# astomodynamics/cddp-cpp

Measured on AMD Instinct MI355X. Metric: trajectories_per_sec, higher is better.
Workload: dtype f64

## Files before the change

cddp-cpp_amd/csrc/capi.hip:

```cpp
#include <algorithm>
#include <chrono>
#include <cmath>
#include <cstdarg>
#include <cstdio>
#include <cstdlib>
#include <cstring>
#include <string>
#include <vector>
#include <map>

#include "launch.hpp"
#include "plant.hpp"
#include "io_kernels.hpp"

static int ladder_strictly_decreasing(const double *a, int n) {
  for (int i = 1; i < n; ++i) if (!(a[i] < a[i - 1])) return 0;
  return n > 0 ? 1 : 0;
}

using namespace cddp_dev;

namespace cddp_dev {
static __global__ void k_gather_records(DevBuf d, cddp_hip_gather_record *out) {
  const int b = blockIdx.x * blockDim.x + threadIdx.x;
// ... 79 lines not shown
  for (int i = 0; i < nu; ++i) Ulog[((size_t)b * steps + k) * nu + i] = Uc[(((size_t)0 * NB + tile) * nu + i) * 64 + lane];
  for (int i = 0; i < nx; ++i) Xlog[((size_t)b * (steps + 1) + k + 1) * nx + i] = Xc[(((size_t)1 * NB + tile) * nx + i) * 64 + lane];
  itlog[(size_t)b * steps + k] = d.iter[b]; stlog[(size_t)b * steps + k] = d.status[b];
}

static __global__ void k_mark_cpu_time(DevBuf d) {
  const int b = blockIdx.x * blockDim.x + threadIdx.x;
  if (b >= d.B || d.phase[b] == PH_DONE) return;
  d.iter[b] += 1; d.status[b] = CDDP_HIP_STATUS_MAX_CPU_TIME; d.phase[b] = PH_DONE;
}

}

int cddp_host_model_eval(int model, int integrator, double dt, const double *params, int nx, int nu, const double *x, const double *u, double *x_next,
                         double *fx, double *fu, double *fxx, double *fuu, double *fux, std::string &err);
int cddp_host_model_params(int model, int nx, int nu, const double *in, double *out, std::string &err);

namespace {

thread_local std::string g_err;
int fail(int code, const char *fmt, ...) {
  char buf[1024];
  va_list ap; va_start(ap, fmt); vsnprintf(buf, sizeof(buf), fmt, ap); va_end(ap);
  g_err = buf;
  return code;
}
}
extern "C" int cddp_hip_internal_set_error(int code, const char *msg) { g_err = msg ? msg : ""; return code; }
extern "C" int cddp_hip_internal_allgather(const void *send, void *recv, size_t bytes_per_rank, void *comm, void *stream);
namespace {
#define HIPCHK(expr)                                                                          \
  do { hipError_t e_ = (expr); if (e_ != hipSuccess)                                           \
      return fail(-10, "%s failed: %s (%s:%d)", #expr, hipGetErrorString(e_), __FILE__, __LINE__); } while (0)

const std::vector<KernelSet> &registry() {
  static std::vector<KernelSet> v = [] {
    std::vector<KernelSet> r;
    register_pendulum(r); register_cartpole(r); register_unicycle(r); register_lti(r);
    register_quadrotor(r); register_quad12(r); register_manipulator(r); register_manip7(r); register_terminal(r); register_statebox(r);
    register_vehicles(r); register_spacecraft(r); register_plants_small(r); register_plants_nx10(r);
    return r;
  }();
  return v;
}

}

struct CuSpec { int lo[3] = {-1, -1, -1}, hi[3] = {-1, -1, -1}; unsigned xcd[3] = {0, 0, 0}; };
struct CuPlan {
  hipStream_t fwd = nullptr, sweep = nullptr;
  hipEvent_t ev[6] = {nullptr, nullptr, nullptr, nullptr, nullptr, nullptr};
  SweepHop hop{nullptr, nullptr, nullptr};
};

struct Inner {
  ProblemDev P;
  DevBuf d;
  const KernelSet *ks = nullptr;
  const Knobs *knob = nullptr;
  Route route;
  int device = 0;
  hipStream_t stream = nullptr;
  bool own_stream = false;
  CuPlan cu;
  std::vector<void *> allocs;
  ProblemDev *dP = nullptr;
  double *d_xref_traj = nullptr;
  unsigned long long *d_launched = nullptr;
  double *d_Xinit = nullptr, *d_Uinit = nullptr;
  bool have_initial = false;
  bool initialized = false;
  bool has_state = false;
  bool initial_dirty = false;
  bool ms_cache_started = false;
  size_t bytes = 0;
  int timing_detail = CDDP_HIP_TIMING_ROLLOUT;
  std::vector<hipEvent_t> ev_pool;
  hipEvent_t ev_begin = nullptr, ev_end = nullptr, ev_poll = nullptr, ev_poll2 = nullptr;
  double *d_head = nullptr, *h_head = nullptr; size_t head_cap = 0;
  int *h_poll = nullptr;
  std::map<unsigned long long, hipGraphExec_t> graphs;
  bool shadow_bufs = false;
  int cs_epoch = 0;
  int n_redo = 0;
  bool last_shadow = false;
  bool ever_solved = false;
  int *h_bad = nullptr;
  bool has_plan = false;
  double *d_xnext = nullptr;
  double *d_log_u = nullptr, *d_log_x = nullptr; int32_t *d_log_it = nullptr, *d_log_st = nullptr; int log_steps = 0;
};

namespace {

template <class T>
int dalloc(Inner *h, T **p, size_t n) {
  if (n == 0) n = 1;
  void *q = nullptr;
  HIPCHK(hipMalloc(&q, n * sizeof(T)));
  HIPCHK(hipMemsetAsync(q, 0, n * sizeof(T), h->stream));
  h->allocs.push_back(q);
  h->bytes += n * sizeof(T);
  *p = (T *)q;
  return 0;
}

int pool_put(ProblemDev &P, int &top, const double *src, int n) {
  if (top + n > kPool) return -1;
  int off = top;
  for (int i = 0; i < n; ++i) P.pool[off + i] = src[i];
  top += n;
  return off;
}

bool model_has_hessians(int model) {
  return model == CDDP_HIP_MODEL_PENDULUM || model == CDDP_HIP_MODEL_CARTPOLE || model == CDDP_HIP_MODEL_UNICYCLE || model == CDDP_HIP_MODEL_LTI ||
         model == CDDP_HIP_MODEL_BICYCLE || model == CDDP_HIP_MODEL_CAR || model == CDDP_HIP_MODEL_MANIPULATOR || model == CDDP_HIP_MODEL_HCW ||
         model == CDDP_HIP_MODEL_QUADROTOR || model == CDDP_HIP_MODEL_QUADROTOR_EULER12 || model == CDDP_HIP_MODEL_MANIPULATOR7 ||
         model == CDDP_HIP_MODEL_EULER_ATTITUDE || model == CDDP_HIP_MODEL_QUATERNION_ATTITUDE || model == CDDP_HIP_MODEL_MRP_ATTITUDE ||
         model == CDDP_HIP_MODEL_SPACECRAFT_LANDING2D ||
         model == CDDP_HIP_MODEL_DUBINS_CAR || model == CDDP_HIP_MODEL_DREYFUS_ROCKET || model == CDDP_HIP_MODEL_ACROBOT || model == CDDP_HIP_MODEL_USV_3DOF ||
         model == CDDP_HIP_MODEL_FORKLIFT || model == CDDP_HIP_MODEL_SPACECRAFT_LINEAR_FUEL || model == CDDP_HIP_MODEL_QUADROTOR_RATE;
}

int fail_no_hessians(int model) {
  if (model == CDDP_HIP_MODEL_SPACECRAFT_NONLINEAR) return fail(-3, "use_ilqr=false: %s", SpacecraftNonlinearModel::kNoHessMsg);
  if (model == CDDP_HIP_MODEL_SPACECRAFT_TWOBODY) return fail(-3, "use_ilqr=false: %s", SpacecraftTwobodyModel::kNoHessMsg);
  return fail(-3, "use_ilqr=false needs the plant's Hessian tensors, which model id %d does not have", model);
}

int flatten(const cddp_hip_problem *p, ProblemDev &P) {
  std::memset(&P, 0, sizeof(P));
  if (p->abi_version != CDDP_HIP_ABI_VERSION) return fail(-2, "ABI version mismatch: got %d want %d", p->abi_version, CDDP_HIP_ABI_VERSION);
  if (p->nx <= 0 || p->nu <= 0 || p->horizon <= 0 || !(p->dt > 0)) return fail(-2, "bad dimensions nx=%d nu=%d N=%d dt=%g", p->nx, p->nu, p->horizon, p->dt);
  if (!p->Q || !p->R || !p->Qf || !p->x_ref) return fail(-2, "objective matrices (Q, R, Qf, x_ref) must be set before solving");
  if (p->solver != CDDP_HIP_SOLVER_CLDDP && p->solver != CDDP_HIP_SOLVER_IPDDP && p->solver != CDDP_HIP_SOLVER_LOGDDP && p->solver != CDDP_HIP_SOLVER_MSIPDDP)
    return fail(-2, "UnknownSolver - No solver registered for id %d", p->solver);
  if (p->solver == CDDP_HIP_SOLVER_MSIPDDP && p->n_constraints > 0 && !(p->nu == 1 || p->nx == p->nu))
    return fail(-3, "MSIPDDP with path constraints is only defined for nu = 1 or nx = nu: the reference adds an (nx x nu) product to its (nu x nx) block Q_ux (msipddp_solver.cpp:1398)");
  if (p->solver == CDDP_HIP_SOLVER_LOGDDP && !(p->options.logddp_relaxed_delta > 0.0))
    return fail(-2, "Relaxation delta must be positive.");
  if (!(p->options.reg_update_factor > 1.0) || !(p->options.reg_max_value > 0.0))
    return fail(-2, "regularization.update_factor must be > 1 and max_value > 0 (got %g, %g)", p->options.reg_update_factor, p->options.reg_max_value);
  if (!p->options.use_ilqr && !model_has_hessians(p->model)) return fail_no_hessians(p->model);
  P.solver = p->solver; P.model = p->model; P.integrator = p->integrator;
  P.nx = p->nx; P.nu = p->nu; P.N = p->horizon; P.dt = p->dt; P.opt = p->options;
  P.ls_rule = p->options.enable_parallel ? CDDP_HIP_LS_BEST_MERIT : CDDP_HIP_LS_FIRST_SUCCESS;
  {
    std::string err;
    if (cddp_host_model_params(p->model, p->nx, p->nu, p->model_params, P.mp, err)) return fail(-2, "%s", err.c_str());
  }
  if (p->model == CDDP_HIP_MODEL_CAR) P.mp[1] = p->dt;
  if (p->model == CDDP_HIP_MODEL_FORKLIFT) P.mp[3] = p->dt;
  if (p->model == CDDP_HIP_MODEL_LTI) {
    if (!p->lti_A || !p->lti_B) return fail(-2, "LTI model needs lti_A and lti_B");
    if (p->nx * p->nx + p->nx * p->nu + 1 > 32) return fail(-3, "LTI dims too large for the device parameter block");
    for (int i = 0; i < p->nx * p->nx; ++i) P.mp[i] = p->lti_A[i];
    for (int i = 0; i < p->nx * p->nu; ++i) P.mp[p->nx * p->nx + i] = p->lti_B[i];
    P.mp[p->nx * p->nx + p->nx * p->nu] = p->dt;
  }
  int top = 0;
  {
    std::vector<double> q((size_t)p->nx * p->nx), r((size_t)p->nu * p->nu);
    for (size_t i = 0; i < q.size(); ++i) q[i] = p->Q[i] * p->dt;
    for (size_t i = 0; i < r.size(); ++i) r[i] = p->R[i] * p->dt;
    P.off_Qdt = pool_put(P, top, q.data(), (int)q.size());
// ... 288 lines not shown
  }
  h->device = device;
  hipError_t e = hipSetDevice(device);
  if (e != hipSuccess) { delete h; return fail(-10, "hipSetDevice: %s", hipGetErrorString(e)); }
  e = make_stream(&h->stream, device, cu ? cu->lo[0] : -1, cu ? cu->hi[0] : -1, cu ? cu->xcd[0] : 0);
  if (e != hipSuccess) { delete h; return fail(-10, "hipStreamCreate: %s", hipGetErrorString(e)); }
  h->own_stream = true;
  if (cu && (cu->lo[1] >= 0 || cu->lo[2] >= 0)) {
    if (cu->lo[1] >= 0) e = make_stream(&h->cu.fwd, device, cu->lo[1], cu->hi[1], cu->xcd[1]);
    if (e == hipSuccess && cu->lo[2] >= 0) e = make_stream(&h->cu.sweep, device, cu->lo[2], cu->hi[2], cu->xcd[2]);
    for (int k = 0; k < 6 && e == hipSuccess; ++k) e = hipEventCreateWithFlags(&h->cu.ev[k], hipEventDisableTiming);
    if (e != hipSuccess) { const int rc_ = fail(-10, "CU-masked stream: %s", hipGetErrorString(e)); in_destroy(h); return rc_; }
    h->cu.hop = SweepHop{h->cu.sweep, h->cu.ev[4], h->cu.ev[5]};
  }

  const ProblemDev &P = h->P;
  DevBuf &d = h->d;
  std::memset(&d, 0, sizeof(d));
  const int B = batch, Bp = (batch + 63) / 64 * 64, N = P.N, nx = P.nx, nu = P.nu, m = P.m;
  d.B = B; d.Bp = Bp; d.NB = Bp / 64; d.N = N; d.n_alphas = P.n_alphas; d.n_slots = P.n_alphas + 1;
  d.ladder_sorted = ladder_strictly_decreasing(P.alphas, P.n_alphas);
  d.ddp = P.opt.use_ilqr ? 0 : 1;
  d.fail_costate_mask = knob.fail_costate;
  d.xcd_map = knob.xcd_map ? 1 : 0;
  d.hist_batch = P.opt.return_iteration_info ? std::min(B, 64) : 0;
  d.hist_cap = std::max(P.opt.max_iterations, 0) + 1;
  d.planeX = (size_t)(N + 1) * nx * Bp; d.planeU = (size_t)N * nu * Bp; d.planeM = (size_t)N * (m > 0 ? m : 0) * Bp;
  const bool ip = (P.solver == CDDP_HIP_SOLVER_IPDDP);
  d.lg = (P.solver == CDDP_HIP_SOLVER_LOGDDP) ? 1 : 0;
  const bool ms = (P.solver == CDDP_HIP_SOLVER_MSIPDDP);
  d.ms = ms ? 1 : 0;
  d.filt_cap = ms ? std::max(P.opt.max_iterations, 0) + 2 : kFilterCap;
#define DA(ptr, n) do { int rc_ = dalloc(h, &(ptr), (size_t)(n)); if (rc_) { in_destroy(h); return rc_; } } while (0)
  DA(d.X, d.planeX * d.n_slots); DA(d.U, d.planeU * d.n_slots);
  if (ip) { DA(d.S, d.planeM * d.n_slots); DA(d.Y, d.planeM * d.n_slots); DA(d.G, d.planeM * d.n_slots); DA(d.Lam, d.planeX * d.n_slots); }
  if (ms) {
    if (m > 0) { DA(d.S, d.planeM * d.n_slots); DA(d.Y, d.planeM * d.n_slots); DA(d.G, d.planeM * d.n_slots);
                 DA(d.ks, (size_t)N * m * Bp); DA(d.ky, (size_t)N * m * Bp); DA(d.Ks, (size_t)N * m * nx * Bp); DA(d.Ky, (size_t)N * m * nx * Bp); }
    DA(d.Lam, d.planeX * d.n_slots); DA(d.F, d.planeX * d.n_slots);
    DA(d.kl, (size_t)N * nx * Bp);
    if (m == 0) DA(d.fac, (size_t)N * (nu * nu + nu + 1) * Bp);
    if (m > 0) { DA(d.ms_res, (size_t)3 * Bp); DA(d.ev, (size_t)d.n_slots * N * P.n_cons * Bp); }
    if (m > 0 && h->ks->ms_cst_size > 0) DA(d.cst, (size_t)N * h->ks->ms_cst_size * Bp);
  }
  DA(d.A, (size_t)N * nx * nx * Bp); DA(d.Bm, (size_t)N * nx * nu * Bp);
  DA(d.K, (size_t)N * nu * nx * Bp); DA(d.k, (size_t)N * nu * Bp);
  if (ip && nx > 8) DA(d.Kt, (size_t)N * (nu * nx + nu) * Bp);
  DA(d.Vx, (size_t)(N + 1) * nx * Bp); DA(d.Vxx, (size_t)(N + 1) * nx * nx * Bp);
  if (ip && h->ks->cst_size > 0) { DA(d.cst, (size_t)N * h->ks->cst_size * Bp); DA(d.dX, (size_t)N * nx * Bp); DA(d.ys, (size_t)N * (m > 0 ? m : 1) * Bp); }
  if (ip && m > 0) { DA(d.ks, (size_t)N * m * Bp); DA(d.ky, (size_t)N * m * Bp); DA(d.Ks, (size_t)N * m * nx * Bp); DA(d.Ky, (size_t)N * m * nx * Bp); }
  double **scal[] = {&d.cost, &d.merit, &d.inf_pr, &d.inf_du, &d.inf_comp, &d.step_norm, &d.alpha_pr, &d.alpha_du, &d.reg, &d.mu,
                     &d.dV0, &d.dV1, &d.phi, &d.theta, &d.filter_theta, &d.apr_max, &d.adu_max};
  for (double **sp : scal) DA(*sp, Bp);
  DA(d.filt, (size_t)2 * d.filt_cap * Bp);
  int **iscal[] = {&d.filt_n, &d.iter, &d.status, &d.phase, &d.cur, &d.n_bwd, &d.n_fwd, &d.bwd_ok};
  for (int **sp : iscal) DA(*sp, Bp);
  double **tr[] = {&d.t_cost, &d.t_merit, &d.t_theta, &d.t_inf_pr, &d.t_inf_comp, &d.t_apr, &d.t_adu, &d.t_ysmin, &d.t_ysmax};
  for (double **sp : tr) DA(*sp, (size_t)d.n_alphas * Bp);
  DA(d.sink, kSinkDoubles);
  DA(d.t_success, (size_t)d.n_alphas * Bp);
  DA(d.t_steps, (size_t)d.n_alphas * Bp); DA(d.n_fwd_steps, Bp); DA(d.cand, Bp);
  if (ip && P.n_cons > 0) DA(d.ev, (size_t)d.n_alphas * N * 2 * P.n_cons * Bp);
  if (d.lg && P.n_cons > 0) DA(d.ev, (size_t)d.n_slots * N * P.n_cons * Bp);
  DA(d.hist, (size_t)std::max(1, d.hist_batch) * d.hist_cap * kHistCols);
  DA(d.hist_n, std::max(1, d.hist_batch));
  if (ip && P.n_term > 0) {
    DA(d.ST, (size_t)8 * Bp); DA(d.YT, (size_t)8 * Bp); DA(d.GT, (size_t)8 * Bp); DA(d.dST, (size_t)8 * Bp); DA(d.dYT, (size_t)8 * Bp);
    DA(d.LamT, (size_t)16 * Bp); DA(d.dLamT, (size_t)16 * Bp);
    DA(d.STt, (size_t)d.n_alphas * 8 * Bp); DA(d.YTt, (size_t)d.n_alphas * 8 * Bp); DA(d.GTt, (size_t)d.n_alphas * 8 * Bp);
    DA(d.LamTt, (size_t)d.n_alphas * 16 * Bp);
    if (P.pT > 0) {
      const bool te_coop = h->ks->te_rec_size > 0 && P.mT == 0 && P.pT + 1 <= h->ks->te_group && P.pT <= P.nx;
      const size_t nv = te_coop ? 16 : (size_t)(P.pT + 1);
      DA(d.te_k, nv * N * nu * Bp); DA(d.te_p, nv * (N + 1) * nx * Bp);
      if (te_coop) {
        DA(d.te_cst, (size_t)N * h->ks->te_rec_size * Bp); DA(d.te_cnt, Bp);
        if (!d.dX) DA(d.dX, (size_t)N * nx * Bp);
        if (!d.ys) DA(d.ys, (size_t)N * (m > 0 ? m : 1) * Bp);
      }
    }
  }
  DA(d.n_active, 1);
  DA(d.win_hist, CDDP_HIP_MAX_ALPHAS + 1);
  DA(h->d_launched, 1);
  DA(h->dP, 1);
  DA(h->d_Xinit, d.planeX); DA(h->d_Uinit, d.planeU);
  if (problem->x_ref_traj) {
    DA(h->d_xref_traj, (size_t)(N + 1) * nx);
    hipMemcpyAsync(h->d_xref_traj, problem->x_ref_traj, sizeof(double) * (N + 1) * nx, hipMemcpyHostToDevice, h->stream);
    d.xref_traj = h->d_xref_traj;
  }
#undef DA
  hipMemcpyAsync(h->dP, &h->P, sizeof(ProblemDev), hipMemcpyHostToDevice, h->stream);
  d.P = h->dP;
  d.launched = h->d_launched;
  resolve_route(h);
  if (shadow_layout(h) && knob.costate != Knobs::kCostateSync && !knob.fail_costate && !knob.graph) {
#define DA(ptr, n) do { int rc_ = dalloc(h, &(ptr), (size_t)(n)); if (rc_) { in_destroy(h); return rc_; } } while (0)
    DA(d.Vx2, (size_t)(N + 1) * nx * Bp); DA(d.Vxx2, (size_t)(N + 1) * nx * nx * Bp);
    DA(d.cs_stampv, Bp); DA(d.cs_old, Bp); DA(d.cs_new, Bp); DA(d.cs_apr, Bp); DA(d.cs_vbuf, Bp); DA(d.cs_bad, 1);
#undef DA
    if (hipHostMalloc((void **)&h->h_bad, sizeof(int)) != hipSuccess) { const int rc_ = fail(-10, "hipHostMalloc failed"); in_destroy(h); return rc_; }
    *h->h_bad = 0;
    h->shadow_bufs = true;
  }
  e = hipStreamSynchronize(h->stream);
  if (e != hipSuccess) { const int rc_ = fail(-10, "device initialisation failed: %s", hipGetErrorString(e)); in_destroy(h); return rc_; }
  *out = h;
  return 0;
}

static int in_destroy(Inner *h) {
  if (h) { for (auto &kv : h->graphs) hipGraphExecDestroy(kv.second); h->graphs.clear(); }
  if (!h) return 0;
  hipSetDevice(h->device);
  hipStreamSynchronize(h->stream);
  if (h->cu.fwd) hipStreamSynchronize(h->cu.fwd);
  if (h->cu.sweep) hipStreamSynchronize(h->cu.sweep);
  free_all(h);
  for (hipEvent_t e : h->ev_pool) hipEventDestroy(e);
  if (h->ev_begin) { hipEventDestroy(h->ev_begin); hipEventDestroy(h->ev_end); }
  if (h->ev_poll) hipEventDestroy(h->ev_poll);
  if (h->ev_poll2) hipEventDestroy(h->ev_poll2);
  if (h->h_poll) hipHostFree(h->h_poll);
  if (h->h_bad) hipHostFree(h->h_bad);
  if (h->d_head) hipFree(h->d_head);
  if (h->h_head) hipHostFree(h->h_head);
  if (h->d_xnext) hipFree(h->d_xnext);
  if (h->d_log_u) { hipFree(h->d_log_u); hipFree(h->d_log_x); hipFree(h->d_log_it); hipFree(h->d_log_st); }
  if (h->own_stream && h->stream) hipStreamDestroy(h->stream);
  if (h->cu.fwd) hipStreamDestroy(h->cu.fwd);
  if (h->cu.sweep) hipStreamDestroy(h->cu.sweep);
  for (hipEvent_t e : h->cu.ev) if (e) hipEventDestroy(e);
  delete h;
  return 0;
}

static int in_set_timing_detail(Inner *h, int detail) {
  if (!h) return fail(-1, "null handle");
  if (detail != CDDP_HIP_TIMING_ROLLOUT && detail != CDDP_HIP_TIMING_ALL && detail != CDDP_HIP_TIMING_SWEEP)
    return fail(-2, "unknown timing detail %d", detail);
  h->timing_detail = detail;
  return 0;
}

static int in_set_stream(Inner *h, void *hip_stream) {
  if (!h) return fail(-1, "null handle");
  hipSetDevice(h->device);
  hipStreamSynchronize(h->stream);
  if (h->own_stream && h->stream) hipStreamDestroy(h->stream);
  h->stream = (hipStream_t)hip_stream;
  h->own_stream = false;
  return 0;
}

static int in_dual_dim(Inner *h) { return h ? h->P.m : -1; }
static int in_batch(Inner *h) { return h ? h->d.B : -1; }

static inline size_t tix(int t, int E, int e, int b, int Bp) { return ((((size_t)t * (Bp / 64) + (size_t)(b >> 6)) * E + e) * 64) + (size_t)(b & 63); }
static void to_soa(const double *src, double *dst, int B, int Bp, int T, int E) {
  for (int b = 0; b < B; ++b)
    for (int t = 0; t < T; ++t)
      for (int e = 0; e < E; ++e) dst[tix(t, E, e, b, Bp)] = src[((size_t)b * T + t) * E + e];
}
static void from_soa(const double *src, double *dst, int B, int Bp, int T, int E) {
  for (int b = 0; b < B; ++b)
    for (int t = 0; t < T; ++t)
      for (int e = 0; e < E; ++e) dst[((size_t)b * T + t) * E + e] = src[tix(t, E, e, b, Bp)];
}

static void from_t4(const double *src, double *dst, int B, int Bp, int T, int E) {
  const size_t NB16 = (size_t)(Bp / 64) * 16;
  for (int b = 0; b < B; ++b)
    for (int t = 0; t < T; ++t)
      for (int e = 0; e < E; ++e) dst[((size_t)b * T + t) * E + e] = src[((((size_t)t * NB16 + (size_t)(b >> 2)) * (size_t)E + (size_t)e) * 4) + (size_t)(b & 3)];
}

static int in_set_initial(Inner *h, const double *x0, const double *U0, const double *X0) {
  if (!h || !x0) return fail(-1, "null argument");
  HIPCHK(hipSetDevice(h->device));
  const DevBuf &d = h->d;
  const int B = d.B, Bp = d.Bp, N = d.N, nx = h->P.nx, nu = h->P.nu;
  std::vector<double> hx((size_t)(N + 1) * nx * Bp, 0.0), hu((size_t)N * nu * Bp, 0.0);
  if (X0) to_soa(X0, hx.data(), B, Bp, N + 1, nx);
  else
    for (int b = 0; b < B; ++b)
      for (int t = 0; t <= N; ++t)
        for (int e = 0; e < nx; ++e) hx[tix(t, nx, e, b, Bp)] = x0[(size_t)b * nx + e];
  for (int b = 0; b < B; ++b)
    for (int e = 0; e < nx; ++e) hx[tix(0, nx, e, b, Bp)] = x0[(size_t)b * nx + e];
  if (U0) to_soa(U0, hu.data(), B, Bp, N, nu);
  HIPCHK(hipMemcpyAsync(h->d_Xinit, hx.data(), hx.size() * sizeof(double), hipMemcpyHostToDevice, h->stream));
  HIPCHK(hipMemcpyAsync(h->d_Uinit, hu.data(), hu.size() * sizeof(double), hipMemcpyHostToDevice, h->stream));
  HIPCHK(hipStreamSynchronize(h->stream));
  h->have_initial = true;
  h->initialized = false;
  h->initial_dirty = true;
  return 0;
}

static int run_initialize(Inner *h) {
  const bool ip = (h->P.solver == CDDP_HIP_SOLVER_IPDDP) || (h->P.solver == CDDP_HIP_SOLVER_MSIPDDP);
  int mode = kInitCold;
  if (h->P.opt.warm_start) mode = h->has_state ? kInitWarmExisting : kInitWarmProvided;
  if (mode == kInitWarmExisting) {
    h->ks->stage(h->d, h->initial_dirty ? 0 : 1, ip ? 1 : 0, h->stream);
    if (h->initial_dirty) { int rc = restore_initial(h); if (rc) return rc; }
// ... 62 lines not shown
    HIPCHK(hipMemcpyAsync(d.X + (size_t)sl * d.planeX, row.data(), row.size() * sizeof(double), hipMemcpyHostToDevice, h->stream));
  HIPCHK(hipMemcpyAsync(h->d_Xinit, row.data(), row.size() * sizeof(double), hipMemcpyHostToDevice, h->stream));
  HIPCHK(hipStreamSynchronize(h->stream));
  h->initialized = false;
  return 0;
}

static int in_set_duals(Inner *h, const double *S, const double *Y) {
  if (!h) return fail(-1, "null handle");
  if (h->P.solver != CDDP_HIP_SOLVER_IPDDP || h->P.m <= 0) return fail(-1, "cddp_hip_set_duals: the problem has no path duals");
  if (!h->has_state) return fail(-1, "cddp_hip_set_duals needs an initialised handle (call cddp_hip_initialize or cddp_hip_solve first)");
  HIPCHK(hipSetDevice(h->device));
  const DevBuf &d = h->d;
  std::vector<double> buf(d.planeM);
  const double *src[2] = {S, Y};
  double *dst[2] = {d.S, d.Y};
  for (int k = 0; k < 2; ++k) {
    if (!src[k]) continue;
    std::fill(buf.begin(), buf.end(), 0.0);
    to_soa(src[k], buf.data(), d.B, d.Bp, d.N, h->P.m);
    for (int sl = 0; sl < d.n_slots; ++sl)
      HIPCHK(hipMemcpyAsync(dst[k] + (size_t)sl * d.planeM, buf.data(), buf.size() * sizeof(double), hipMemcpyHostToDevice, h->stream));
    HIPCHK(hipStreamSynchronize(h->stream));
  }
  return 0;
}

static int in_set_barrier_state(Inner *h, const double *mu, const double *reg) {
  if (!h) return fail(-1, "null handle");
  if (!h->has_state) return fail(-1, "cddp_hip_set_barrier_state needs an initialised handle (call cddp_hip_initialize or cddp_hip_solve first)");
  HIPCHK(hipSetDevice(h->device));
  const DevBuf &d = h->d;
  if (mu) {
    if (h->P.solver != CDDP_HIP_SOLVER_IPDDP) return fail(-1, "cddp_hip_set_barrier_state: mu is an IPDDP quantity");
    for (int b = 0; b < d.B; ++b) if (!(mu[b] > 0.0)) return fail(-2, "barrier parameter of trajectory %d must be positive (got %g)", b, mu[b]);
    HIPCHK(hipMemcpyAsync(d.mu, mu, sizeof(double) * d.B, hipMemcpyHostToDevice, h->stream));
  }
  if (reg) {
    for (int b = 0; b < d.B; ++b) if (!(reg[b] >= 0.0)) return fail(-2, "regularisation of trajectory %d must be non-negative (got %g)", b, reg[b]);
    HIPCHK(hipMemcpyAsync(d.reg, reg, sizeof(double) * d.B, hipMemcpyHostToDevice, h->stream));
  }
  HIPCHK(hipStreamSynchronize(h->stream));
  return 0;
}

static int in_set_terminal(Inner *h, const double *S_T, const double *Y_T, const double *Lambda_T) {
  if (!h) return fail(-1, "null handle");
  if (h->P.n_term <= 0) return fail(-1, "cddp_hip_set_terminal: the problem has no terminal constraints");
  if (!h->has_state) return fail(-1, "cddp_hip_set_terminal needs an initialised handle");
  HIPCHK(hipSetDevice(h->device));
  const DevBuf &d = h->d;
  struct { const double *host; double *dev; int n; } items[] = {{S_T, d.ST, h->P.mT}, {Y_T, d.YT, h->P.mT}, {Lambda_T, d.LamT, h->P.pT}};
  for (auto &it : items) {
    if (!it.host || it.n <= 0) continue;
    std::vector<double> buf((size_t)it.n * d.Bp, 0.0);
    for (int b = 0; b < d.B; ++b) for (int i = 0; i < it.n; ++i) buf[(size_t)i * d.Bp + b] = it.host[(size_t)b * it.n + i];
    HIPCHK(hipMemcpyAsync(it.dev, buf.data(), buf.size() * sizeof(double), hipMemcpyHostToDevice, h->stream));
    HIPCHK(hipStreamSynchronize(h->stream));
  }
  return 0;
}

static int in_backward(Inner *h, int32_t *ok) {
  if (!h) return fail(-1, "null handle");
  HIPCHK(hipSetDevice(h->device));
  if (!h->initialized) { int rc = in_initialize(h); if (rc) return rc; }
  h->ks->derivs(h->d, h->route, 1, h->stream);
  h->ks->backward(h->d, h->route, h->P.solver, 1, 0, h->stream);
  HIPCHK(hipGetLastError());
  if (ok) HIPCHK(hipMemcpyAsync(ok, h->d.bwd_ok, sizeof(int) * h->d.B, hipMemcpyDeviceToHost, h->stream));
  HIPCHK(hipStreamSynchronize(h->stream));
  return 0;
}

static int in_forward(Inner *h, const double *alphas, int n_alphas, cddp_hip_trial *trials) {
  if (!h || !alphas || !trials) return fail(-1, "null argument");
  if (n_alphas <= 0 || n_alphas > h->d.n_alphas) return fail(-1, "n_alphas must be in [1, %d] (the handle's ladder size)", h->d.n_alphas);
  HIPCHK(hipSetDevice(h->device));
  ProblemDev tmp = h->P;
  for (int i = 0; i < n_alphas; ++i) tmp.alphas[i] = alphas[i];
  HIPCHK(hipMemcpyAsync(h->dP, &tmp, sizeof(ProblemDev), hipMemcpyHostToDevice, h->stream));
  DevBuf dcall = h->d;
  dcall.ladder_sorted = ladder_strictly_decreasing(tmp.alphas, h->d.n_alphas);
  h->ks->forward(dcall, h->route, h->P.solver, 0, n_alphas, PH_FWD1, 1, 0, h->stream);
  h->ks->costate(dcall, h->route, h->P.solver, 0, n_alphas, PH_FWD1, 1, 0, h->stream);
  HIPCHK(hipGetLastError());
  const DevBuf &d = h->d;
  const size_t n = (size_t)n_alphas * d.Bp;
  std::vector<double> c(n), mf(n), th(n), ipr(n), ic(n), ap(n), ad(n);
  std::vector<int> su(n);
  HIPCHK(hipMemcpyAsync(c.data(), d.t_cost, n * 8, hipMemcpyDeviceToHost, h->stream));
  HIPCHK(hipMemcpyAsync(mf.data(), d.t_merit, n * 8, hipMemcpyDeviceToHost, h->stream));
  HIPCHK(hipMemcpyAsync(th.data(), d.t_theta, n * 8, hipMemcpyDeviceToHost, h->stream));
  HIPCHK(hipMemcpyAsync(ipr.data(), d.t_inf_pr, n * 8, hipMemcpyDeviceToHost, h->stream));
  HIPCHK(hipMemcpyAsync(ic.data(), d.t_inf_comp, n * 8, hipMemcpyDeviceToHost, h->stream));
  HIPCHK(hipMemcpyAsync(ap.data(), d.t_apr, n * 8, hipMemcpyDeviceToHost, h->stream));
  HIPCHK(hipMemcpyAsync(ad.data(), d.t_adu, n * 8, hipMemcpyDeviceToHost, h->stream));
  HIPCHK(hipMemcpyAsync(su.data(), d.t_success, n * 4, hipMemcpyDeviceToHost, h->stream));
  HIPCHK(hipMemcpyAsync(h->dP, &h->P, sizeof(ProblemDev), hipMemcpyHostToDevice, h->stream));
  HIPCHK(hipStreamSynchronize(h->stream));
  for (int b = 0; b < d.B; ++b)
    for (int a = 0; a < n_alphas; ++a) {
      cddp_hip_trial &t = trials[(size_t)b * n_alphas + a];
      const size_t i = (size_t)a * d.Bp + b;
      t.alpha = alphas[a]; t.alpha_pr = ap[i]; t.alpha_du = ad[i]; t.cost = c[i]; t.merit_function = mf[i];
      t.theta = th[i]; t.inf_pr = ipr[i]; t.inf_comp = ic[i]; t.success = (su[i] == 1) ? 1 : 0; t._pad = 0;
    }
  return 0;
}

struct SolveRun {
  Inner *h = nullptr;
  bool want_stats = false;
  int conc = 1;
  int detail = -1;
  std::vector<int> ev_slot;
  size_t ev_used = 0;
  int launches = 0, outer = 0, it = 0, max_it = 0, na = 0;
  bool two_stage_marks = false, first_rule = true, pinned = false, one_stage = true, done = false, cpu_time_hit = false, use_graph = false;
  int k1 = 1, k_cap = 1, k_cap2 = 1;
  bool shadow = false, force_sync = false, pre_has_state = false, redo_needed = false;
  int stamp0 = 0;
  long waves_all = 0, per_alpha_waves = 1, two_stage_max_waves = 768;
  std::vector<int> hist_now, hist_prev;
  static constexpr int kPollWords = CDDP_HIP_MAX_ALPHAS + 2;
  hipEvent_t poll_evs[2] = {nullptr, nullptr};
  int win_enq = 0, win_dig = 0, win_it[2] = {0, 0};
  int outstanding() const { return win_enq - win_dig; }
  bool ran_ahead = false;
  int post_poll(hipStream_t s) {
    const int slot = win_enq & 1;
    HIPCHK(hipMemcpyAsync(h->h_poll + slot * kPollWords, h->d.n_active, sizeof(int), hipMemcpyDeviceToHost, s));
    HIPCHK(hipMemcpyAsync(h->h_poll + slot * kPollWords + 1, h->d.win_hist, sizeof(int) * (na + 1), hipMemcpyDeviceToHost, s));
    HIPCHK(hipEventRecord(poll_evs[slot], s));
    win_it[slot] = it;
    ++win_enq;
    return 0;
  }
  std::chrono::steady_clock::time_point wall0;
  hipEvent_t fwd_wait = nullptr, fwd_done = nullptr;

  void mark(int point) {
    if (detail < 0) return;
    const bool want = detail == CDDP_HIP_TIMING_ALL ||
                      (detail == CDDP_HIP_TIMING_ROLLOUT && (point == 1 || point == 2 || (two_stage_marks && (point == 3 || point == 4)))) ||
                      (detail == CDDP_HIP_TIMING_SWEEP && (point == 0 || point == 1));
    if (!want) return;
    if (ev_used == h->ev_pool.size()) {
      hipEvent_t e;
      if ((h->knob->event_fence ? hipEventCreate(&e) : hipEventCreateWithFlags(&e, hipEventDisableSystemFence)) != hipSuccess) return;
      h->ev_pool.push_back(e);
    }
    const size_t slot = (size_t)6 * (size_t)(outer - 1) + (size_t)point;
    if (ev_slot.size() <= slot) ev_slot.resize(slot + 1, -1);
    hipEventRecord(h->ev_pool[ev_used], h->stream);
    ev_slot[slot] = (int)ev_used++;
  }

  void adapt_ladder(int window_iters) {
    if (pinned) return;
    long total = 0;
    std::vector<long> hd(na + 1);
    for (int a = 0; a <= na; ++a) { hd[a] = (long)hist_now[a] - (long)hist_prev[a]; total += hd[a]; }
    hist_prev = hist_now;
    if (total <= 0) return;
    const long allow = std::max(1L, (long)window_iters / 4);
    int kq = na;
    long tail = hd[na];
    for (int k = na - 1; k >= 1; --k) {
      tail += hd[k];
      if (tail <= allow) kq = k; else break;
    }
    if (kq >= na - 1) {
      if (waves_all <= 2048) { one_stage = true; }
      else { one_stage = false; k1 = k_cap2; }
    } else {
      one_stage = false; k1 = std::max(1, std::min(kq + h->knob->ls_margin, k_cap));
      if (waves_all <= 2048 && (long)k1 * per_alpha_waves > two_stage_max_waves) one_stage = true;
      const long small_cap = (h->P.solver == CDDP_HIP_SOLVER_LOGDDP || h->P.solver == CDDP_HIP_SOLVER_MSIPDDP) ? 2048 : 1024;
      if (waves_all <= small_cap && h->P.nx <= 8 && h->knob->ls_small_frac * k1 > na) one_stage = true;
    }
    if (h->knob->debug_ladder) {
      std::fprintf(stderr, "[ladder] it=%d total=%ld kq=%d -> %s k1=%d hist:", outer, total, kq, one_stage ? "one" : "two", k1);
      for (int a = 0; a <= na; ++a) std::fprintf(stderr, " %ld", hd[a]);
      std::fprintf(stderr, "\n");
    }
  }

  int begin(Inner *h_, bool stats_, int conc_) {
    h = h_; want_stats = stats_; conc = std::max(1, conc_);
    const ProblemDev &P = h->P;
    const DevBuf &d = h->d;
    hipStream_t s = h->stream;
    const KernelSet *ks = h->ks;
    max_it = P.opt.max_iterations;
    first_rule = (P.ls_rule == CDDP_HIP_LS_FIRST_SUCCESS);
    na = d.n_alphas;
    use_graph = h->knob->graph;
    if (use_graph && conc > 1) {
      static bool said = false;
      if (!said) { said = true; std::fprintf(stderr, "[cddp_hip] CDDP_HIP_GRAPH=1: graph replay does not keep the CU-masked streams' partition; the tile groups share the whole chip\n"); }
    }
    detail = (want_stats && !use_graph) ? h->timing_detail : -1;
    if (!h->ev_begin) { HIPCHK(hipEventCreate(&h->ev_begin)); HIPCHK(hipEventCreate(&h->ev_end)); }
    if (!h->ev_poll) { HIPCHK(hipEventCreateWithFlags(&h->ev_poll, hipEventDisableTiming)); HIPCHK(hipEventCreateWithFlags(&h->ev_poll2, hipEventDisableTiming)); }
    poll_evs[0] = h->ev_poll; poll_evs[1] = h->ev_poll2;
    win_enq = win_dig = 0; ran_ahead = false;
    if (!h->h_poll) HIPCHK(hipHostMalloc((void **)&h->h_poll, sizeof(int) * 2 * kPollWords));
    HIPCHK(hipMemsetAsync(h->d_launched, 0, sizeof(unsigned long long), s));
    HIPCHK(hipEventRecord(h->ev_begin, s));
    pre_has_state = h->has_state;
    shadow = !force_sync && shadow_eligible(h, conc) && max_it > 0;
    redo_needed = false;
    h->last_shadow = shadow; h->ever_solved = true;
    if (shadow) HIPCHK(hipMemsetAsync(h->d.cs_bad, 0, sizeof(int), s));
    stamp0 = h->cs_epoch;
    { int rc = run_initialize(h); if (rc) return rc; }
    launches = 1; outer = 0; it = 0; done = false;
    *h->h_poll = d.B;
    waves_all = (long)conc * (long)((d.B + 63) / 64) * na * (((P.solver == CDDP_HIP_SOLVER_IPDDP && (ks->cst_size > 0 || (d.te_cst && P.m > 0))) || P.solver == CDDP_HIP_SOLVER_MSIPDDP || P.solver == CDDP_HIP_SOLVER_LOGDDP) ? 2 : 1);
    const bool force_two = h->knob->ls_stages == '2', force_one = h->knob->ls_stages == '1';
    const long per_alpha = std::max(1L, waves_all / std::max(1, na));
    per_alpha_waves = per_alpha;
    two_stage_max_waves = h->knob->ls_two_max_waves;
    k_cap = (int)std::max(1L, std::min((long)na - 1, 1024 / per_alpha));
    k_cap2 = (int)std::max(1L, std::min((long)na - 1, 2048 / per_alpha));
    const int k_forced = h->knob->ls_first;
    pinned = !first_rule || na == 1 || force_one || force_two || (k_forced >= 1 && k_forced < na);
    one_stage = !first_rule || na == 1 || force_one || (waves_all <= 2048 && !force_two);
    k1 = force_two ? 1 : k_cap2;
    if (k_forced >= 1 && k_forced < na && !force_one && first_rule) { one_stage = false; k1 = k_forced; }
    hist_now.assign(na + 1, 0); hist_prev.assign(na + 1, 0);
    HIPCHK(hipMemsetAsync(d.win_hist, 0, sizeof(int) * (CDDP_HIP_MAX_ALPHAS + 1), s));
    wall0 = std::chrono::steady_clock::now();
    if (max_it <= 0) { ks->update(d, h->route, 2, 0, 1, 1, s); ++launches; done = true; }
    return 0;
  }

  void enqueue_iteration(int last) {
    const ProblemDev &P = h->P;
    if (shadow) {
      DevBuf &hd = h->d;
      hd.Vx_prev = hd.Vx; hd.Vxx_prev = hd.Vxx;
      std::swap(hd.Vx, hd.Vx2); std::swap(hd.Vxx, hd.Vxx2);
      hd.cs_vsel ^= 1;
    }
    DevBuf dsh = h->d;
    if (shadow) {
      h->cs_epoch += 2;
      dsh.cs_mode = 1; dsh.cs_stamp = h->cs_epoch + 1; dsh.cs_want = dsh.cs_stamp - 2;
      dsh.cs_fail_stamp = h->knob->fail_shadow > 0 ? stamp0 + 2 * h->knob->fail_shadow + 1 : 0;
    }
    const DevBuf &d = dsh;
    hipStream_t s = h->stream;
    const KernelSet *ks = h->ks;
    const Route &r = h->route;
    hipStream_t sf = h->cu.fwd ? h->cu.fwd : s;
    auto to_fwd = [&](int k) { if (sf != s) { order_check(hipEventRecord(h->cu.ev[k], s)); order_check(hipStreamWaitEvent(sf, h->cu.ev[k], 0)); } };
    auto from_fwd = [&](int k) { if (sf != s) { order_check(hipEventRecord(h->cu.ev[k], sf)); order_check(hipStreamWaitEvent(s, h->cu.ev[k], 0)); } };
    two_stage_marks = !one_stage;
    mark(0);
    ks->derivs(d, r, 0, s);
    tl_sweep_hop = h->cu.sweep ? &h->cu.hop : nullptr;
    if (shadow && outer > 1) { dsh.cs_extra = ks->shadow_extra(d, r); ks->backward(dsh, r, P.solver, 0, 1, s); dsh.cs_extra = 0; }
    else ks->backward(d, r, P.solver, 0, 1, s);
    tl_sweep_hop = nullptr;
    mark(1);
    to_fwd(0);
    if (fwd_wait) hipStreamWaitEvent(sf, fwd_wait, 0);
    if (one_stage) {
      ks->forward(d, r, P.solver, 0, na, PH_FWD1, 0, first_rule ? 1 : 0, sf);
      if (fwd_done) hipEventRecord(fwd_done, sf);
      from_fwd(1);
      mark(2);
      if (!shadow) ks->costate(d, r, P.solver, 0, na, PH_FWD1, 0, first_rule ? 1 : 2, s);
      ks->update(d, r, 1, na, last, 1, s);
      mark(3);
      launches += shadow ? 3 : 4;
    } else {
      ks->forward(d, r, P.solver, 0, k1, PH_FWD1, 0, 1, sf);
      from_fwd(1);
      mark(2);
      if (!shadow) ks->costate(d, r, P.solver, 0, k1, PH_FWD1, 0, 1, s);
      if (shadow) {
        DevBuf d1 = dsh;
        d1.cs_stamp = h->cs_epoch;
        ks->update(d1, r, 1, k1, last, 0, s);
        d1.cs_want = d1.cs_stamp; d1.Vx_prev = d1.Vx; d1.Vxx_prev = d1.Vxx;
        ks->shadow_flush(d1, nullptr, s);
      } else
      ks->update(d, r, 1, k1, last, 0, s);
      mark(3);
      to_fwd(2);
      ks->forward(d, r, P.solver, k1, na - k1, PH_FWD2, 0, 1, sf);
      if (fwd_done) hipEventRecord(fwd_done, sf);
      from_fwd(3);
      mark(4);
      if (!shadow) ks->costate(d, r, P.solver, k1, na - k1, PH_FWD2, 0, 1, s);
      ks->update(d, r, 2, na, last, 1, s);
      mark(5);
      launches += shadow ? 5 : 6;
    }
  }
  bool polled_iteration(int i) const { return i % h->knob->poll_every == 0 || i == max_it || (i <= 2 && !pinned); }

  int advance_graph() {
    const hipStream_t s = h->stream;
    int w = 0;
    while (it + w < max_it) { ++w; if (polled_iteration(it + w)) break; }
    if (w == 0) { done = true; return 0; }
    const int last = (it + w == max_it) ? 1 : 0;
    const unsigned long long key = ((unsigned long long)(one_stage ? 0 : k1) << 16) | ((unsigned long long)w << 4) | (unsigned long long)last;
    auto f = h->graphs.find(key);
    if (f == h->graphs.end()) {
      hipGraph_t g = nullptr; hipGraphExec_t ge = nullptr;
      const int launches0 = launches;
      HIPCHK(hipStreamBeginCapture(s, hipStreamCaptureModeThreadLocal));
      for (int j = 1; j <= w; ++j) enqueue_iteration((j == w) ? last : 0);
      HIPCHK(hipStreamEndCapture(s, &g));
      HIPCHK(hipGraphInstantiate(&ge, g, nullptr, nullptr, 0));
      hipGraphDestroy(g);
      launches = launches0;
      f = h->graphs.emplace(key, ge).first;
    }
    { const int l0 = launches; for (int j = 0; j < w; ++j) launches += one_stage ? 4 : 6; (void)l0; }
    HIPCHK(hipGraphLaunch(f->second, s));
    it += w; outer += w;
    { int rc = post_poll(s); if (rc) return rc; }
    return 1;
  }

  int advance(int max_new = 1 << 30) {
    if (done) return 0;
    int enq = 0;
    const ProblemDev &P = h->P;
    const DevBuf &d = h->d;
    hipStream_t s = h->stream;
    if (use_graph && !(P.opt.max_cpu_time > 0.0)) return advance_graph();
    while (it < max_it) {
      ++it;
      if (P.opt.max_cpu_time > 0.0) {
        HIPCHK(hipStreamSynchronize(s));
        const double el_ms = (double)std::chrono::duration_cast<std::chrono::milliseconds>(std::chrono::steady_clock::now() - wall0).count();
        if (el_ms > P.opt.max_cpu_time * 1000.0) {
          hipLaunchKernelGGL(k_mark_cpu_time, dim3((d.B + 255) / 256), dim3(256), 0, s, d);
          ++launches; done = true; cpu_time_hit = true;
          return 0;
        }
      }
      ++outer;
      const int last = (it == max_it) ? 1 : 0;
      enqueue_iteration(last);
      if (polled_iteration(it)) {
        { int rc = post_poll(s); if (rc) return rc; }
        return 1;
      }
      if (++enq >= max_new) return 2;
    }
    done = true;
    return 0;
  }

  int complete_poll() {
    const int kPollEvery = h->knob->poll_every;
    if (outstanding() <= 0) return 0;
    const int slot = win_dig & 1;
    HIPCHK(hipEventSynchronize(poll_evs[slot]));
    ++win_dig;
    const int *w = h->h_poll + slot * kPollWords;
    const int pit = win_it[slot];
    if (w[0] == 0 || pit >= max_it) { done = true; win_dig = win_enq; return 0; }
    for (int a = 0; a <= na; ++a) hist_now[a] = w[1 + a];
    adapt_ladder(pit <= 2 ? 1 : (pit == kPollEvery ? 2 : kPollEvery));
    return 0;
  }

  int flush() {
    const DevBuf &d = h->d;
    hipStream_t s = h->stream;
    if (shadow) {
      DevBuf df = h->d, dm = h->d;
      df.cs_mode = 1; df.cs_want = h->cs_epoch > stamp0 ? h->cs_epoch + 1 : 0; df.Vx_prev = df.Vx; df.Vxx_prev = df.Vxx;
      df.cs_fail_stamp = h->knob->fail_shadow > 0 ? stamp0 + 2 * h->knob->fail_shadow + 1 : 0;
      h->ks->shadow_flush(df, &dm, s);
      launches += df.cs_want > 0 ? 2 : 1;
      HIPCHK(hipMemsetD32Async((hipDeviceptr_t)d.cs_vbuf, d.cs_vsel, (size_t)d.Bp, s));
      HIPCHK(hipMemcpyAsync(h->h_bad, d.cs_bad, sizeof(int), hipMemcpyDeviceToHost, s));
    }
    return 0;
  }

  int finish(cddp_hip_stats *stats) {
    const DevBuf &d = h->d;
    hipStream_t s = h->stream;
    HIPCHK(hipEventRecord(h->ev_end, s));
    HIPCHK(hipStreamSynchronize(s));
    HIPCHK(hipGetLastError());
    if (shadow && *h->h_bad != 0) { redo_needed = true; return 0; }
    if (tl_order_error != hipSuccess) {
      const hipError_t oe = tl_order_error; tl_order_error = hipSuccess;
      return fail(-10, "stream ordering (event record / wait) failed during the solve: %s", hipGetErrorString(oe));
    }
    if (!stats) return 0;
    std::memset(stats, 0, sizeof(*stats));
    float ms = 0;
    hipEventElapsedTime(&ms, h->ev_begin, h->ev_end);
    stats->solve_ms = ms;
    auto span = [&](size_t it0, int pa, int pb) -> double {
      const size_t ia = it0 * 6 + (size_t)pa, ib = it0 * 6 + (size_t)pb;
      if (ib >= ev_slot.size() || ev_slot[ia] < 0 || ev_slot[ib] < 0) return 0.0;
      float v = 0;
      hipEventElapsedTime(&v, h->ev_pool[ev_slot[ia]], h->ev_pool[ev_slot[ib]]);
      return v;
    };
    for (size_t it0 = 0; it0 * 6 < ev_slot.size(); ++it0) {
      stats->backward_ms += span(it0, 0, 1);
      stats->forward_ms += span(it0, 1, 2) + span(it0, 3, 4);
      stats->update_ms += span(it0, 2, 3) + span(it0, 4, 5);
    }
    if (detail != CDDP_HIP_TIMING_ALL) stats->update_ms = 0.0;
    if (detail == CDDP_HIP_TIMING_ROLLOUT) stats->backward_ms = 0.0;
    if (detail == CDDP_HIP_TIMING_SWEEP) stats->forward_ms = 0.0;
    stats->timing_detail = detail;
    std::vector<int> nb(d.B), nf(d.B), itv(d.B), stv(d.B), nst(d.B);
    HIPCHK(hipMemcpy(nst.data(), d.n_fwd_steps, sizeof(int) * d.B, hipMemcpyDeviceToHost));
    HIPCHK(hipMemcpy(nb.data(), d.n_bwd, sizeof(int) * d.B, hipMemcpyDeviceToHost));
    HIPCHK(hipMemcpy(nf.data(), d.n_fwd, sizeof(int) * d.B, hipMemcpyDeviceToHost));
    HIPCHK(hipMemcpy(itv.data(), d.iter, sizeof(int) * d.B, hipMemcpyDeviceToHost));
    HIPCHK(hipMemcpy(stv.data(), d.status, sizeof(int) * d.B, hipMemcpyDeviceToHost));
    for (int b = 0; b < d.B; ++b) {
      stats->sweeps += nb[b]; stats->rollouts += nf[b]; stats->traj_iterations += itv[b]; stats->rollout_steps += nst[b];
      if (stv[b] == CDDP_HIP_STATUS_OPTIMAL || stv[b] == CDDP_HIP_STATUS_ACCEPTABLE) stats->n_converged++;
    }
    unsigned long long nl = 0;
    HIPCHK(hipMemcpy(&nl, h->d_launched, sizeof(nl), hipMemcpyDeviceToHost));
    stats->rollouts_launched = (int64_t)nl;
    stats->outer_iterations = outer; stats->kernel_launches = launches;
    return 0;
  }
};

static int fetch(Inner *h, const double *dev, size_t n, std::vector<double> &host) {
  host.resize(n);
  HIPCHK(hipMemcpy(host.data(), dev, n * sizeof(double), hipMemcpyDeviceToHost));
  return 0;
}

static int in_get_results(Inner *h, cddp_hip_result *r) {
  if (!h || !r) return fail(-1, "null argument");
  HIPCHK(hipSetDevice(h->device));
  HIPCHK(hipStreamSynchronize(h->stream));
  const DevBuf &d = h->d;
  const int B = d.B;
  std::vector<double> v[10];
  const double *src[10] = {d.cost, d.merit, d.inf_pr, d.inf_du, d.inf_comp, d.mu, d.reg, d.alpha_pr, d.alpha_du, d.step_norm};
  for (int i = 0; i < 10; ++i) { int rc = fetch(h, src[i], B, v[i]); if (rc) return rc; }
  std::vector<int> it(B), st(B), nb(B), nf(B);
  HIPCHK(hipMemcpy(it.data(), d.iter, sizeof(int) * B, hipMemcpyDeviceToHost));
  HIPCHK(hipMemcpy(st.data(), d.status, sizeof(int) * B, hipMemcpyDeviceToHost));
  HIPCHK(hipMemcpy(nb.data(), d.n_bwd, sizeof(int) * B, hipMemcpyDeviceToHost));
  HIPCHK(hipMemcpy(nf.data(), d.n_fwd, sizeof(int) * B, hipMemcpyDeviceToHost));
  for (int b = 0; b < B; ++b) {
    r[b].final_objective = v[0][b]; r[b].merit_function = v[1][b]; r[b].inf_pr = v[2][b]; r[b].inf_du = v[3][b];
    r[b].inf_comp = v[4][b]; r[b].barrier_mu = v[5][b]; r[b].regularization = v[6][b]; r[b].alpha_pr = v[7][b];
    r[b].alpha_du = v[8][b]; r[b].step_norm = v[9][b]; r[b].iterations = it[b]; r[b].status = st[b];
    r[b].n_backward = nb[b]; r[b].n_forward = nf[b];
  }
  return 0;
}

static int fetch_current(Inner *h, const double *base, size_t plane, int T, int E, double *out) {
  const DevBuf &d = h->d;
  std::vector<int> cur(d.B);
  HIPCHK(hipMemcpy(cur.data(), d.cur, sizeof(int) * d.B, hipMemcpyDeviceToHost));
  std::vector<char> need(d.n_slots, 0);
  for (int b = 0; b < d.B; ++b) need[cur[b]] = 1;
  std::vector<double> buf;
  for (int s = 0; s < d.n_slots; ++s) {
    if (!need[s]) continue;
    int rc = fetch(h, base + (size_t)s * plane, plane, buf);
// ... 280 lines not shown
  for (Inner *q : h->g) {
    if (q->stream == h->user_stream) continue;
    HIPCHK(hipEventRecord(h->ev_join, q->stream));
    HIPCHK(hipStreamWaitEvent(h->user_stream, h->ev_join, 0));
  }
  return 0;
}

}

static int drive_runs(SolveRun *run, int n) {
  for (;;) {
    bool any = false;
    for (int k = 0; k < n; ++k) {
      SolveRun &r = run[k];
      const Inner *g = r.h;
      const int ra = (g->P.opt.max_cpu_time > 0.0 || r.use_graph || r.it < g->knob->poll_every) ? 0 : g->knob->run_ahead;
      if (!r.done && r.outstanding() == 0) { int rc = r.advance(); if (rc < 0) return rc; r.ran_ahead = false; any = true; }
      else if (!r.done && r.outstanding() == 1 && ra > 0 && !r.ran_ahead) { int rc = r.advance(ra); if (rc < 0) return rc; r.ran_ahead = true; any = true; }
      else if (r.outstanding() > 0) { int rc = r.complete_poll(); if (rc) return rc; r.ran_ahead = r.outstanding() > 0; any = true; }
    }
    if (!any) break;
  }
  return 0;
}

extern "C" {

int cddp_hip_create(const cddp_hip_problem *problem, int batch, int device, cddp_hip_handle **out) {
  if (!problem || !out) return fail(-1, "null argument");
  if (batch <= 0) return fail(-1, "batch must be positive");
  int conc = 1, part = 1;
  double ladder[CDDP_HIP_MAX_ALPHAS];
  const int n_ladder = cddp_hip_build_alphas(&problem->options, ladder, CDDP_HIP_MAX_ALPHAS);
  cddp_hip_handle *h = new cddp_hip_handle();
  const Knobs &knob = h->knob;
  if (knob.fail_costate) std::fprintf(stderr, "[cddp_hip] TEST HOOK active: CDDP_HIP_TEST_FAIL_COSTATE=%d discards line-search trials -- results are not the solver's\n", knob.fail_costate);
  const int tiles = (batch + 63) / 64, ng = pick_groups(knob, batch, n_ladder, problem->solver, &conc, &part);
  h->B = batch; h->device = device; h->conc = conc;
  int t0 = 0;
  for (int k = 0; k < ng; ++k) {
    const int nt = tiles / ng + (k < tiles % ng ? 1 : 0);
    const int first = t0 * 64, last = std::min(batch, (t0 + nt) * 64);
    t0 += nt;
    if (last <= first) continue;
    Inner *q = nullptr;
    CuSpec cus;
    bool have_cu = cu_spec_for_group(knob, k, &cus);
    if (!have_cu && part > 1) {
      const int w = device_cu_count(device) / part / 8 * 8;
      if (w >= 16) { cus.lo[0] = (k % part) * w; cus.hi[0] = cus.lo[0] + w; have_cu = true; }
    }
    int rc = in_create(problem, last - first, device, knob, have_cu ? &cus : nullptr, &q);
    if (rc) { for (Inner *p : h->g) in_destroy(p); delete h; return rc; }
    h->g.push_back(q); h->b0.push_back(first);
  }
  const ProblemDev &P = h->g[0]->P;
  h->nx = P.nx; h->nu = P.nu; h->N = P.N; h->m = P.m; h->mT = P.mT; h->pT = P.pT;
  *out = h;
  return 0;
}

int cddp_hip_destroy(cddp_hip_handle *h) {
  if (!h) return 0;
  for (Inner *q : h->g) in_destroy(q);
  if (h->ev_fork) { hipEventDestroy(h->ev_fork); hipEventDestroy(h->ev_join); }
  for (int k = 0; k < 2; ++k) if (h->ev_pp[k]) hipEventDestroy(h->ev_pp[k]);
  if (h->d_send) hipFree(h->d_send);
  delete h;
  return 0;
}

int cddp_hip_num_groups(cddp_hip_handle *h) { return h ? (int)h->g.size() : -1; }
int cddp_hip_costate_mode(cddp_hip_handle *h) {
  if (!h) return -1;
  for (Inner *q : h->g) if (!(q->ever_solved ? q->last_shadow : shadow_eligible(q, std::max(1, std::min(h->conc, (int)h->g.size()))))) return 0;
  return 1;
}
int cddp_hip_costate_redos(cddp_hip_handle *h) {
  if (!h) return -1;
  int n = 0;
  for (Inner *q : h->g) n += q->n_redo;
  return n;
}
int cddp_hip_concurrency(cddp_hip_handle *h) { return h ? std::max(1, std::min(h->conc, (int)h->g.size())) : -1; }

int cddp_hip_set_timing_detail(cddp_hip_handle *h, int detail) {
  if (!h) return fail(-1, "null handle");
  for (Inner *q : h->g) { int rc = in_set_timing_detail(q, detail); if (rc) return rc; }
  return 0;
}

int cddp_hip_set_stream(cddp_hip_handle *h, void *hip_stream) {
  if (!h) return fail(-1, "null handle");
  h->user_stream = (hipStream_t)hip_stream; h->have_user_stream = true;
  if (h->g.size() == 1) return in_set_stream(h->g[0], hip_stream);
  return 0;
}

int cddp_hip_dual_dim(cddp_hip_handle *h) { return h ? h->m : -1; }
int cddp_hip_batch(cddp_hip_handle *h) { return h ? h->B : -1; }

#define OFF(ptr, stride) ((ptr) ? (ptr) + (size_t)h->b0[gi_] * (size_t)(stride) : nullptr)
#define FOR_GROUPS(call) do { if (!h) return fail(-1, "null handle"); { int rc_ = fork_from_user(h); if (rc_) return rc_; } \
    for (size_t gi_ = 0; gi_ < h->g.size(); ++gi_) { Inner *q = h->g[gi_]; (void)q; int rc_ = (call); if (rc_) return rc_; } \
    return join_to_user(h); } while (0)

int cddp_hip_set_initial(cddp_hip_handle *h, const double *x0, const double *U0, const double *X0) {
  if (!x0) return fail(-1, "null argument");
  FOR_GROUPS(in_set_initial(q, OFF(x0, h->nx), OFF(U0, h->N * h->nu), OFF(X0, (h->N + 1) * h->nx)));
}
int cddp_hip_initialize(cddp_hip_handle *h) { FOR_GROUPS(in_initialize(q)); }
int cddp_hip_set_options(cddp_hip_handle *h, const cddp_hip_options *opt) { FOR_GROUPS(in_set_options(q, opt)); }
int cddp_hip_set_initial_state(cddp_hip_handle *h, const double *x0) {
  if (!x0) return fail(-1, "null argument");
  FOR_GROUPS(in_set_initial_state(q, OFF(x0, h->nx)));
}
int cddp_hip_forget_solver_state(cddp_hip_handle *h) {
  if (!h) return fail(-1, "null handle");
  for (Inner *q : h->g) { q->has_state = false; q->initialized = false; }
  return 0;
}
int cddp_hip_set_duals(cddp_hip_handle *h, const double *S, const double *Y) { FOR_GROUPS(in_set_duals(q, OFF(S, h->N * h->m), OFF(Y, h->N * h->m))); }
int cddp_hip_set_barrier_state(cddp_hip_handle *h, const double *mu, const double *reg) { FOR_GROUPS(in_set_barrier_state(q, OFF(mu, 1), OFF(reg, 1))); }
int cddp_hip_set_terminal(cddp_hip_handle *h, const double *S_T, const double *Y_T, const double *Lambda_T) {
  FOR_GROUPS(in_set_terminal(q, OFF(S_T, h->mT), OFF(Y_T, h->mT), OFF(Lambda_T, h->pT)));
}
int cddp_hip_backward(cddp_hip_handle *h, int32_t *ok) { FOR_GROUPS(in_backward(q, OFF(ok, 1))); }
int cddp_hip_forward(cddp_hip_handle *h, const double *alphas, int n_alphas, cddp_hip_trial *trials) {
  if (!alphas || !trials) return fail(-1, "null argument");
  FOR_GROUPS(in_forward(q, alphas, n_alphas, OFF(trials, n_alphas)));
}
int cddp_hip_get_results(cddp_hip_handle *h, cddp_hip_result *r) { if (!r) return fail(-1, "null argument"); FOR_GROUPS(in_get_results(q, OFF(r, 1))); }
int cddp_hip_get_plan_head(cddp_hip_handle *h, double *u0, double *x1) { FOR_GROUPS(in_get_plan_head(q, OFF(u0, h->nu), OFF(x1, h->nx))); }
int cddp_hip_get_trajectory(cddp_hip_handle *h, double *X, double *U) { FOR_GROUPS(in_get_trajectory(q, OFF(X, (h->N + 1) * h->nx), OFF(U, h->N * h->nu))); }
int cddp_hip_get_gains(cddp_hip_handle *h, double *K, double *k) { FOR_GROUPS(in_get_gains(q, OFF(K, h->N * h->nu * h->nx), OFF(k, h->N * h->nu))); }
int cddp_hip_get_value(cddp_hip_handle *h, double *Vx, double *Vxx) { FOR_GROUPS(in_get_value(q, OFF(Vx, (h->N + 1) * h->nx), OFF(Vxx, (h->N + 1) * h->nx * h->nx))); }
int cddp_hip_get_linearization(cddp_hip_handle *h, double *A, double *Bm) { FOR_GROUPS(in_get_linearization(q, OFF(A, h->N * h->nx * h->nx), OFF(Bm, h->N * h->nx * h->nu))); }
int cddp_hip_get_duals(cddp_hip_handle *h, double *S, double *Y, double *G) {
  FOR_GROUPS(in_get_duals(q, OFF(S, h->N * h->m), OFF(Y, h->N * h->m), OFF(G, h->N * h->m)));
}
int cddp_hip_get_costates(cddp_hip_handle *h, double *Lambda, int32_t *rows) {
  if (!h) return fail(-1, "null handle");
  const int r = (h->g.empty() || !h->g[0]) ? 0 : costate_rows(h->g[0]);
  FOR_GROUPS(in_get_costates(q, OFF(Lambda, r * h->nx), rows));
}
int cddp_hip_get_terminal(cddp_hip_handle *h, double *S_T, double *Y_T, double *G_T, double *Lambda_T, int32_t *dims) {
  FOR_GROUPS(in_get_terminal(q, OFF(S_T, h->mT), OFF(Y_T, h->mT), OFF(G_T, h->mT), OFF(Lambda_T, h->pT), dims));
}
int cddp_hip_get_backward_scalars(cddp_hip_handle *h, double *dV, double *reg) { FOR_GROUPS(in_get_backward_scalars(q, OFF(dV, 2), OFF(reg, 1))); }
int cddp_hip_history_capacity(cddp_hip_handle *h) { return h ? in_history_capacity(h->g[0]) : -1; }
int cddp_hip_get_history(cddp_hip_handle *h, int hist_batch, double *hist, int32_t *counts) {
  if (!h) return fail(-1, "null handle");
  return in_get_history(h->g[0], hist_batch, hist, counts);
}
int cddp_hip_write_gather_records_device(cddp_hip_handle *h, void *device_ptr) {
  if (!device_ptr) return fail(-1, "null argument");
  FOR_GROUPS(in_write_gather_records_device(q, (char *)device_ptr + (size_t)h->b0[gi_] * sizeof(cddp_hip_gather_record)));
}
#undef FOR_GROUPS
#undef OFF

int cddp_hip_allgather_results(cddp_hip_handle *h, void *comm, int world, int shard_capacity, void *recv_device) {
  if (!h || !recv_device) return fail(-1, "null argument");
  if (world <= 0) return fail(-1, "world must be positive");
  if (shard_capacity < h->B) return fail(-1, "shard_capacity %d is smaller than this rank's batch %d", shard_capacity, h->B);
// ... 498 lines not shown
```

cddp-cpp_amd/csrc/dev_types.hpp:

```cpp
#pragma once
#include <stdint.h>
#include <stddef.h>
#include "../../include/cddp_hip.h"

namespace cddp_dev {

constexpr int kMaxCons = 4;
constexpr int kMaxTerms = 2;
constexpr int kPool = 1024;
constexpr int kFilterCap = 8;
constexpr int kHistCols = 9;

enum Phase : int { PH_ACTIVE = 0, PH_FWD1 = 1, PH_FWD2 = 2, PH_DONE = 3 };

struct ConDev {
  int kind, dim, dual_dim, offset;
  int off_lower, off_upper, off_center, off_A, off_b;
  int _pad;
  double scale, radius;
};

struct TermDev {
  int kind, dim, offset;
  int off_target, off_A, off_b;
};

struct ProblemDev {
  int solver, model, integrator, nx, nu, N, m, n_cons;
  int n_term, mT, pT, ls_rule, n_alphas, clddp_box;
  int has_xref_traj, _pad;
  double dt;
  double mp[32];
  cddp_hip_options opt;
  ConDev cons[kMaxCons];
  TermDev terms[kMaxTerms];
  int off_Qdt, off_Rdt, off_Qf, off_xref;
  double alphas[CDDP_HIP_MAX_ALPHAS];
  double pool[kPool];
};

constexpr int kLS = 64;

constexpr int kSinkDoubles = 1024 * 64;

struct DevBuf {
  int B, Bp, N, n_slots, n_alphas, hist_batch, hist_cap, NB;
  int fail_costate_mask;
  const ProblemDev *P;
  const double *xref_traj;
  double *X, *U, *S, *Y, *G, *Lam;
  size_t planeX, planeU, planeM;
  double *A, *Bm, *K, *k, *Vx, *Vxx, *ks, *ky, *Ks, *Ky;
  double *ST, *YT, *GT, *dST, *dYT, *LamT, *dLamT;
  double *STt, *YTt, *GTt, *LamTt;
  double *te_k, *te_p;
  double *te_cst;
  int *te_cnt;
  double *cost, *merit, *inf_pr, *inf_du, *inf_comp, *step_norm, *alpha_pr, *alpha_du, *reg, *mu;
  double *dV0, *dV1, *phi, *theta, *filter_theta, *apr_max, *adu_max;
  double *filt;
  int *filt_n, *iter, *status, *phase, *cur, *n_bwd, *n_fwd, *bwd_ok;
  double *t_cost, *t_merit, *t_theta, *t_inf_pr, *t_inf_comp, *t_apr, *t_adu;
  double *t_ysmin, *t_ysmax;
  int ddp;
  double *sink;
  int *t_success;
  int *t_steps;
  int *n_fwd_steps;
  double *cst;
  double *ys;
  double *Kt;
  double *dX;
  double *ev;
  double *hist;
  int *hist_n;
  int *n_active;
  int ev_valid;
  int *win_hist;
  unsigned long long *launched;
  int *cand;
  int t4;
  int lg;
  int ms;
  int ms_fresh;
  int filt_cap;
  double *F;
  double *kl;
  double *fac;
  int ladder_sorted;
  double *ms_res;
  int xcd_map;
  double *Vx2, *Vxx2;
  const double *Vx_prev, *Vxx_prev;
  int *cs_stampv, *cs_old, *cs_new;
  double *cs_apr;
  int *cs_vbuf;
  int *cs_bad;
  int cs_mode;
  int cs_stamp;
  int cs_want;
  int cs_fail_stamp;
  int cs_vsel;
  int cs_extra;
};

}
```

cddp-cpp_amd/csrc/kernels_coop.hpp:

```cpp
#pragma once
#include "kernels_lean.hpp"
#include "kernels_logddp.hpp"
#include <type_traits>
#include <utility>

namespace cddp_dev {

#define GI(t, E, e) (((((size_t)(t)) * (size_t)d.NB + (size_t)(b >> 6)) * (E) + (e)) * 64 + (size_t)(b & 63))

template <class Model>
struct CoopCfg {
  static constexpr int NX = Model::NX, NU = Model::NU;
  static constexpr int G = NX <= 4 ? 4 : (NX <= 8 ? 8 : 16);
  static constexpr int TPW = 64 / G;
  static constexpr int oT1 = 0, oT2 = oT1 + NX * NX, oKK = oT2 + NU * NX, oQux = oKK + NU * NX, oVn = oQux + NU * NX,
                       oVx = oVn + NX * NX, oDx = oVx + NX, RAW = oDx + NX;
  static constexpr int STRIDE = (RAW + 31) / 32 * 32 + 4;
};

DEV void lds_sync() { asm volatile("s_waitcnt lgkmcnt(0)" ::: "memory"); }

template <int P> DEV double quad_bcast(double v) {
  constexpr int ctrl = P | (P << 2) | (P << 4) | (P << 6);
  const int lo = __builtin_amdgcn_update_dpp(0, __double2loint(v), ctrl, 0xF, 0xF, false);
// ... 98 lines not shown
        if (!front && expect < i_min) return -1;
        int v = 0;
        if (leader) v = front ? __hip_atomic_fetch_add(&s_take, 1, __ATOMIC_RELAXED, __HIP_MEMORY_SCOPE_WORKGROUP)
                              : __hip_atomic_fetch_sub(&s_take, 1 << 16, __ATOMIC_RELAXED, __HIP_MEMORY_SCOPE_WORKGROUP);
        v = __builtin_amdgcn_readfirstlane(v);
        const int f = v & 0xffff, bk = v >> 16;
        if (f > bk) return -1;
        expect = bk - 1;
        return front ? f : bk;
      };
      struct PIn { double x[NX], y[M], sv[M], g[M], kk[NU], KK[NU * NX], uj[NU], ys[M]; };
      auto pload = [&](int i, PIn &r) {
        const int t = i * RC::SPB + so;
        if (need && i >= 0 && t < N) {
          ld<NX>(Xc + GI(t, NX, 0), kLS, r.x);
          ld<M>(Yc + GI(t, M, 0), kLS, r.y);
          ld<M>(Sc + GI(t, M, 0), kLS, r.sv);
          ld<M>(Gc + GI(t, M, 0), kLS, r.g);
          ld<NU>(d.k + GI(t, NU, 0), kLS, r.kk);
          ld<NU * NX>(d.K + GI(t, NU * NX, 0), kLS, r.KK);
          if constexpr (Cons::NEEDS_U) ld<NU>(Uc + GI(t, NU, 0), kLS, r.uj);
          ld<M>(d.ys + GI(t, M, 0), kLS, r.ys);
        }
      };
      auto pproc = [&](const int i, const PIn &in, const int inext) {
        const int t = i * RC::SPB + so;
        const bool valid = need && t < N;
        double ky[M], ksv[M], Ky[M * NX], Ksm[M * NX], ysv[M];
        if (valid) {
#pragma unroll
          for (int r = 0; r < M; ++r) ysv[r] = in.ys[r];
          post_rows<Model, Cons, true>(P, in.x, in.uj, in.y, in.sv, in.g, in.kk, in.KK, mu, ky, ksv, ysv, Ky, Ksm);
          st<M>(d.ky + GI(t, M, 0), kLS, ky);
          st<M>(d.ks + GI(t, M, 0), kLS, ksv);
        }
        const int last = (i + 1) * RC::SPB < N ? (i + 1) * RC::SPB : N;
        wait_ge(&s_dxprod, last);
        if (valid) {
          const double *slot = s_ring + ((size_t)(t % RD) * C::TPW + tl) * NX;
          double dx[NX];
#pragma unroll
          for (int k = 0; k < NX; ++k) dx[k] = slot[k];
          double apr = 1.0, adu = 1.0;
          post_caps<NX, M>(ky, ksv, Ky, Ksm, in.sv, in.y, dx, tau, apr, adu);
          if (apr < 1.0) { const unsigned long long v = (unsigned long long)__double_as_longlong(apr >= 0.0 ? apr : 0.0); run_apr = v < run_apr ? v : run_apr; }
          if (adu < 1.0) { const unsigned long long v = (unsigned long long)__double_as_longlong(adu >= 0.0 ? adu : 0.0); run_adu = v < run_adu ? v : run_adu; }
        }
        if (front) {
          asm volatile("s_waitcnt lgkmcnt(0)" ::: "memory");
          __hip_atomic_store(&s_cur[hidx], inext >= 0 ? inext : kNone, __ATOMIC_RELAXED, __HIP_MEMORY_SCOPE_WORKGROUP);
        }
      };
      PIn pa, pb;
      int i0 = take();
      if (front) __hip_atomic_store(&s_cur[hidx], i0 >= 0 ? i0 : kNone, __ATOMIC_RELAXED, __HIP_MEMORY_SCOPE_WORKGROUP);
      pload(i0, pa);
      while (i0 >= 0) {
        const int i1 = take();
        pload(i1, pb);
        PIPELINE_FENCE();
        pproc(i0, pa, i1);
        if (i1 < 0) break;
        const int i2 = take();
        pload(i2, pa);
        PIPELINE_FENCE();
        pproc(i1, pb, i2);
        i0 = i2;
      }
      if (need) {
        __hip_atomic_fetch_min(&s_aprv[tl], run_apr, __ATOMIC_RELAXED, __HIP_MEMORY_SCOPE_WORKGROUP);
        __hip_atomic_fetch_min(&s_aduv[tl], run_adu, __ATOMIC_RELAXED, __HIP_MEMORY_SCOPE_WORKGROUP);
      }
      asm volatile("s_waitcnt lgkmcnt(0)" ::: "memory");
    }
  };
  if constexpr (ROLES) {
    if (d.cs_extra > 0 && (int)blockIdx.x >= (int)gridDim.x - d.cs_extra) {
      const int nw = d.cs_extra * (1 + NH), items = d.NB * (N + 1);
      for (int it = ((int)blockIdx.x - ((int)gridDim.x - d.cs_extra)) * (1 + NH) + wave; it < items; it += nw)
        costate_shadow_item<NX>(d, (it % d.NB) * 64 + lane, it / d.NB);
      return;
    }
    if (blockIdx.x == 0 && threadIdx.x == 0 && !force) *d.n_active = 0;
    const bool act = (b < d.B) && (force || d.phase[b] == PH_ACTIVE);
    if (__builtin_amdgcn_ballot_w64(act) == 0ull) return;
    if (threadIdx.x == 0) {
      s_ret = 0; s_verdict = 1; s_hdone = 0; s_phase2 = 0; s_dxprod = 0; s_pdone = 0;
      s_take = (((N + RC::SPB - 1) / RC::SPB - 1) << 16);
#pragma unroll
      for (int i = 0; i < NH; ++i) s_cur[i] = 0;
#pragma unroll
      for (int i = 0; i < RB; ++i) s_ready[i] = 0;
    }
    __syncthreads();
    const int nblk = (N + RC::SPB - 1) / RC::SPB;
    if (helper) {
      const int hidx = wave - 1;
      const int so = lane / C::TPW;
      if (hidx == 0) { ROLES_STAMP(8); ROLES_ZERO(13); }
      const int cur = act ? d.cur[b] : 0;
      const double *Xc = d.X + (size_t)cur * d.planeX;
      const double *Uc = d.U + (size_t)cur * d.planeU;
      const double *Sc = d.S + (size_t)cur * d.planeM;
      const double *Yc = d.Y + (size_t)cur * d.planeM;
      const double *Gc = d.G + (size_t)cur * d.planeM;
      const double mu = act ? d.mu[b] : 1.0;
      constexpr int M = Cons::M;
      struct HIn { double x[NX], u[NU], y[M], sv[M], g[M]; };
      auto hload = [&](int j, HIn &r) {
        const int t = N - 1 - (j * RC::SPB + so);
        if (act && j < nblk && t >= 0) {
          ld<NX>(Xc + GI(t, NX, 0), kLS, r.x);
          ld<NU>(Uc + GI(t, NU, 0), kLS, r.u);
          ld<M>(Yc + GI(t, M, 0), kLS, r.y);
          ld<M>(Sc + GI(t, M, 0), kLS, r.sv);
          ld<M>(Gc + GI(t, M, 0), kLS, r.g);
        }
      };
      for (int pass = 0;; ++pass) {
        auto hstep = [&](const int j, const HIn &in, HIn &nxt) {
          if (j >= nblk) return;
          hload(j + NH, nxt);
          PIPELINE_FENCE();
          const int gj = pass * nblk + j;
          const int t = N - 1 - (j * RC::SPB + so);
          const bool valid = act && t >= 0;
          double A[NX * NX], Bq[NX * NU], c[CST], ysr[M];
          if (valid) condense_eval<Model, Cons, true>(P, xrt, t, in.x, in.u, in.y, in.sv, in.g, mu, A, Bq, c, ysr);
          if (gj >= RB) wait_ge(&s_ret, (gj - RB + 1) * RC::SPB);
          if (valid) {
            double *r = s_ring + ((size_t)((gj % RB) * RC::SPB + so) * C::TPW + tl) * RC::RECP;
#pragma unroll
            for (int i = 0; i < NX * NX; ++i) r[RC::oA + i] = A[i];
#pragma unroll
            for (int i = 0; i < NX * NU; ++i) r[RC::oB + i] = Bq[i];
#pragma unroll
            for (int i = 0; i < CST; ++i) r[RC::oC + i] = c[i];
            if (pass == 0) {
#pragma unroll
              for (int i = 0; i < NX * NX; ++i) d.A[GI(t, NX * NX, i)] = A[i];
#pragma unroll
              for (int i = 0; i < NX * NU; ++i) d.Bm[GI(t, NX * NU, i)] = Bq[i];
              st<M>(d.ys + GI(t, M, 0), kLS, ysr);
            }
          }
          asm volatile("s_waitcnt lgkmcnt(0)" ::: "memory");
          __hip_atomic_store(&s_ready[gj % RB], gj + 1, __ATOMIC_RELAXED, __HIP_MEMORY_SCOPE_WORKGROUP);
          if (hidx == 0 && gj == 0) ROLES_STAMP(9);
        };
        HIn ha, hb;
        hload(hidx, ha);
        for (int j = hidx; j < nblk; j += 2 * NH) { hstep(j, ha, hb); hstep(j + NH, hb, ha); }
        if (hidx == 0 && pass == 0) ROLES_STAMP(10);
        if (wait_ge(&s_verdict, pass + 2) >= RC::kDone) break;
      }
      __builtin_amdgcn_fence(__ATOMIC_RELEASE, "workgroup");
      if (lane == 0) __hip_atomic_fetch_add(&s_hdone, 1, __ATOMIC_RELAXED, __HIP_MEMORY_SCOPE_WORKGROUP);
      if (wait_ge(&s_phase2, 1) != 1) return;
      __builtin_amdgcn_fence(__ATOMIC_ACQUIRE, "workgroup");
      if (hidx == 0) ROLES_STAMP(11);
      post_phase(so, act && s_need[tl] != 0, mu, cur, true, hidx);
      if (hidx == 0) ROLES_STAMP(12);
      if (lane == 0) __hip_atomic_fetch_add(&s_pdone, 1, __ATOMIC_RELAXED, __HIP_MEMORY_SCOPE_WORKGROUP);
      return;
    }
  }
// ... 1942 lines not shown
```

cddp-cpp_amd/csrc/kernels_lean.hpp:

```cpp
#pragma once
#include "kernels.hpp"

namespace cddp_dev {

#define GI(t, E, e) (((((size_t)(t)) * (size_t)d.NB + (size_t)(b >> 6)) * (E) + (e)) * 64 + (size_t)(b & 63))

template <class Model, class Cons>
struct CstLayout {
  static constexpr int NX = Model::NX, NU = Model::NU;
  static constexpr int CX = 0, CU = CX + NX, WQYU = CU + NU, QYUSIR = WQYU + NU * NU, IPR = QYUSIR + NU, ICOMP = IPR + 1;
  static constexpr int WQYX = ICOMP + 1, QYXSIR = WQYX + NU * NX, WXQYX = QYXSIR + NX;
  static constexpr int SIZE = Cons::HAS_X ? (WXQYX + NX * NX) : WQYX;
};

template <class Model, class Cons, bool WITH_DERIVS>
DEV void condense_eval(const ProblemDev *__restrict__ P, const double *__restrict__ xrt, const int t, const double *x, const double *u,
                       const double *y, const double *s, const double *g, const double mu, double *A, double *Bq, double *c,
                       double *ys_out = nullptr) {
  constexpr int NX = Model::NX, NU = Model::NU, M = Cons::M;
  typedef Objective<NX, NU> Obj;
  typedef CstLayout<Model, Cons> L;
  const double s_floor = dmax(mu * 1e-3, kEpsSlack);
  double Qyx[M * NX], Qyu[M * NU];
  if constexpr (WITH_DERIVS) {
// ... 532 lines not shown
  constexpr int NX = Model::NX;
  const int b = blockIdx.x * 64 + threadIdx.x;
  const int t = blockIdx.y;
  if (b >= d.B) return;
  if (!force && d.phase[b] != phase_req) return;
  const int cur = d.cur[b];
  constexpr int NT = NX * (NX + 1) / 2;
  double xo[NX], lo[NX], vx[NX], vt[NT];
  ld<NX>(d.X + (size_t)cur * d.planeX + GI(t, NX, 0), kLS, xo);
  ld<NX>(d.Lam + (size_t)cur * d.planeX + GI(t, NX, 0), kLS, lo);
  ld<NX>(d.Vx + GI(t, NX, 0), kLS, vx);
  costate_load_triangle<NX>(d.Vxx + GI(t, NX * NX, 0), vt);
  int a_lo = a0, a_hi = a0 + na;
  if (first_only != 0) {
    const int only = first_only == 2 ? d.cand[b] : first_surviving_trial(d, a0, na, b);
    if (only < 0) return;
    a_lo = only; a_hi = only + 1;
  }
  for (int a = a_lo; a < a_hi; ++a) {
    const size_t ti = (size_t)a * d.Bp + b;
    if (!d.t_success[ti]) continue;
    const int slot = trial_slot(cur, a);
    const double a_pr = d.t_apr[ti];
    double xn[NX], lam[NX];
    ld<NX>(d.X + (size_t)slot * d.planeX + GI(t, NX, 0), kLS, xn);
    const bool finite = costate_row_eval<NX>(lo, vx, vt, xo, xn, a_pr, lam);
    if (!finite || ((d.fail_costate_mask >> a) & 1)) d.t_success[ti] = 2;
    else st<NX>(d.Lam + (size_t)slot * d.planeX + GI(t, NX, 0), kLS, lam);
  }
}

template <int NX>
DEV void costate_shadow_item(const DevBuf &d, const int b, const int t) {
  if (b >= d.B) return;
  if (d.cs_stampv[b] != d.cs_want) return;
  const int cur = d.cs_old[b], slot = d.cs_new[b];
  const double a_pr = d.cs_apr[b];
  double xo[NX], lo[NX], vx[NX], xn[NX], lam[NX], vt[NX * (NX + 1) / 2];
  ld<NX>(d.X + (size_t)cur * d.planeX + GI(t, NX, 0), kLS, xo);
  ld<NX>(d.Lam + (size_t)cur * d.planeX + GI(t, NX, 0), kLS, lo);
  ld<NX>(d.Vx_prev + GI(t, NX, 0), kLS, vx);
  costate_load_triangle<NX>(d.Vxx_prev + GI(t, NX * NX, 0), vt);
  ld<NX>(d.X + (size_t)slot * d.planeX + GI(t, NX, 0), kLS, xn);
  const bool finite = costate_row_eval<NX>(lo, vx, vt, xo, xn, a_pr, lam);
  if (!finite || (d.cs_fail_stamp != 0 && d.cs_fail_stamp == (d.cs_want | 1))) *d.cs_bad = 1;
  else st<NX>(d.Lam + (size_t)slot * d.planeX + GI(t, NX, 0), kLS, lam);
}

template <class Model>
__global__ __launch_bounds__(64) void k_costate_flush(DevBuf d) {
  costate_shadow_item<Model::NX>(d, blockIdx.x * 64 + threadIdx.x, blockIdx.y);
}

template <int NX>
__global__ __launch_bounds__(64) void k_value_merge(DevBuf d) {
  const int b = blockIdx.x * 64 + threadIdx.x, t = blockIdx.y;
  if (b >= d.B || d.cs_vbuf[b] == d.cs_vsel) return;
  double vx[NX], vxx[NX * NX];
  ld<NX>(d.Vx2 + GI(t, NX, 0), kLS, vx);
  ld<NX * NX>(d.Vxx2 + GI(t, NX * NX, 0), kLS, vxx);
  st<NX>(d.Vx + GI(t, NX, 0), kLS, vx);
  st<NX * NX>(d.Vxx + GI(t, NX * NX, 0), kLS, vxx);
}
#ifdef CDDP_K4_TIMING
__device__ unsigned long long g_k4_times[16384 * 4];
#define K4_TIME_BEGIN const unsigned long long k4_t0 = wall_clock64();
#define K4_TIME_END(role, steps) do { if (lane == 0) { const size_t k4_i = ((size_t)blockIdx.y * gridDim.x + blockIdx.x) * 4 + (role) * 2; \
    g_k4_times[k4_i] = wall_clock64() - k4_t0; g_k4_times[k4_i + 1] = (unsigned long long)(steps); } } while (0)
#else
#define K4_TIME_BEGIN
#define K4_TIME_END(role, steps)
#endif
template <int NX, int NU> struct RollIn { double x[NX], u[NU]; };
template <int NX> struct RollOut { double xn[NX]; };
template <class Model>
__device__ __attribute__((noinline)) RollOut<Model::NX> roll_step_checked(int integrator, double dt, const double *mp, RollIn<Model::NX, Model::NU> in) {
  RollOut<Model::NX> o;
  Stepper<Model>::step(integrator, dt, mp, in.x, in.u, o.xn);
  return o;
}

template <class Model, class Cons, bool TERM = false, int NC = 1>
__global__ __launch_bounds__(64 * (1 + NC)) void k_forward_ipddp_pc(DevBuf d, const ProblemDev *__restrict__ Pk, const double *__restrict__ xrt,
                                                                    int a0, int phase_req, int force) {
  constexpr int NX = Model::NX, NU = Model::NU, M = Cons::M;
  typedef Objective<NX, NU> Obj;
  static_assert(M > 0, "two-role rollout is for path-constrained problems");
  constexpr int RW = 2 * NX + NU;
  constexpr int kRing = RW <= 10 ? 8 : (RW <= 20 ? 4 : 2);
  __shared__ double s_ring[kRing * RW * 64];
  static_assert(NC == 1 || NC == 2, "one or two consumer waves");
  __shared__ int s_prod;
  __shared__ int s_consv[2];
  [[maybe_unused]] __shared__ int s_abort;
  [[maybe_unused]] __shared__ int s_done1;
  constexpr int kL2 = NC > 1 ? 64 : 1;
  [[maybe_unused]] __shared__ int s_pfail[kL2], s_palive[kL2];
  [[maybe_unused]] __shared__ double s_pmax[4 * kL2];
  [[maybe_unused]] __shared__ double s_prun[kL2];
  __shared__ int s_pstat[64];
  __shared__ double s_pcost[64];
  __shared__ double s_xN[TERM ? NX * 64 : 1];
  __shared__ double s_obj[Obj::kStage];
  const int lane = threadIdx.x & 63;
  K4_TIME_BEGIN
  const int wave = __builtin_amdgcn_readfirstlane((int)threadIdx.x) >> 6;
  const bool producer = wave == 0;
  [[maybe_unused]] const int ci = NC > 1 ? wave - 1 : 0;
  int *const s_cons = &s_consv[0];
  const int b = blockIdx.x * 64 + lane;
  const int a = a0 + blockIdx.y;
  const ProblemDev *__restrict__ P = Pk;
  const cddp_hip_options &o = P->opt;
  const int N = d.N;
  const bool active = (b < d.B) && (force || d.phase[b] == phase_req);
  if (__builtin_amdgcn_ballot_w64(active) == 0ull) return;
  if (producer) { s_pstat[lane] = N + 2; if (lane == 0) { s_prod = 0; s_consv[0] = 0; s_consv[1] = 0; if constexpr (NC > 1) { s_abort = 0x7fffffff; s_done1 = 0; } } }
  Obj::stage(P, s_obj, (int)threadIdx.x, 64 * (1 + NC));
  __syncthreads();
  const int bb = (b < d.B) ? b : 0;
  const int cur = (b < d.B) ? d.cur[b] : 0;
  const int slot = trial_slot(cur, a);
  const double *Xc = d.X + (size_t)cur * d.planeX;
  const double alpha = P->alphas[a];
  const double a_pr = dmin(alpha, d.apr_max[bb]);
  auto wait_ge = [&](int *ctr, int need) -> int {
    int v;
    while ((v = __hip_atomic_load(ctr, __ATOMIC_RELAXED, __HIP_MEMORY_SCOPE_WORKGROUP)) < need) __builtin_amdgcn_s_sleep(1);
    asm volatile("" ::: "memory");
    return v;
  };
  const int kAbort = 2 * N + kRing;

  if (producer) {
    double *Xn = d.X + (size_t)slot * d.planeX;
    double *Un = d.U + (size_t)slot * d.planeU;
    const double *Uc = d.U + (size_t)cur * d.planeU;
    bool alive = active;
    double x[NX];
    ld<NX>(Xc + GI(0, NX, 0), kLS, x);
    st<NX>(Xn + GI(0, NX, 0), kLS, x);
    struct StepIn { double xo[NX], uo[NU], kk[NU], KK[NU * NX]; };
    const size_t rs1 = (size_t)d.NB * 64;
    const double *ld_X = Xc + GI(0, NX, 0), *ld_U = Uc + GI(0, NU, 0), *ld_k = d.k + GI(0, NU, 0), *ld_K = d.K + GI(0, NU * NX, 0);
    double *st_U = Un + GI(0, NU, 0), *st_X = Xn + GI(1, NX, 0);
    auto load_step = [&](int tt, StepIn &r) {
      ld<NX>(Xc + GI(tt, NX, 0), kLS, r.xo);
      ld<NU>(Uc + GI(tt, NU, 0), kLS, r.uo);
      ld<NU>(d.k + GI(tt, NU, 0), kLS, r.kk);
      ld<NU * NX>(d.K + GI(tt, NU * NX, 0), kLS, r.KK);
    };
    auto load_row = [&](StepIn &r) {
      ld<NX>(ld_X, kLS, r.xo);
      ld<NU>(ld_U, kLS, r.uo);
      ld<NU>(ld_k, kLS, r.kk);
      ld<NU * NX>(ld_K, kLS, r.KK);
    };
    auto advance_ld = [&](const int t) {
      const size_t s = t + 1 < N ? rs1 : 0;
      ld_X += s * NX; ld_U += s * NU; ld_k += s * NU; ld_K += s * (NU * NX);
    };
    DynCtx dc;
    dc.load(P->integrator, P->dt, P->mp);
    [[maybe_unused]] typename Obj::Ctx oc_p;
    [[maybe_unused]] double run_cost_p = 0.0;
    if constexpr (NC > 1) Obj::load_staged(P, oc_p, s_obj);
    auto prime = [&]() {
      double z[NX];
#pragma unroll
      for (int i = 0; i < NX; ++i) z[i] = 0.0;
      st<NU>(Un + GI(0, NU, 0), kLS, z);
      st<NX>(Xn + GI(1, NX, 0), kLS, z);
    };
    constexpr bool kPing = sizeof(StepIn) <= 40 * sizeof(double);
    constexpr bool kEarly = !kPing && sizeof(StepIn) <= 96 * sizeof(double);
    constexpr bool kChunkP = !kPing && !kEarly;
    struct PChunk { double K[NX], uo, kk; };
    auto load_pchunk = [&](int tt, const int i, PChunk &c) {
      ld<NX>(d.K + GI(tt, NU * NX, i * NX), kLS, c.K);
      c.uo = Uc[GI(tt, NU, i)]; c.kk = d.k[GI(tt, NU, i)];
    };
    PChunk pk0, pk1;
    double xo_c[NX];
    constexpr bool kFlagged = kPing && HasTrigPolicy<Model>::value && NC == 1;
    auto step = [&](auto integ, const int t, StepIn &cs, StepIn &nxt) {
      constexpr int INTEG = decltype(integ)::value;
      if constexpr (kPing) {
        advance_ld(t);
        load_row(nxt);
      }
      PIPELINE_FENCE();
      double dx[NX], u[NU], xn[NX];
      bool finite = true;
      if constexpr (kChunkP) {
#pragma unroll
        for (int i = 0; i < NX; ++i) dx[i] = x[i] - xo_c[i];
#pragma unroll
        for (int i = 0; i < NU; ++i) {
          if (i + 1 < NU) { if ((i & 1) == 0) load_pchunk(t, i + 1, pk1); else load_pchunk(t, i + 1, pk0); }
          __builtin_amdgcn_sched_barrier(0);
          const PChunk &c = (i & 1) == 0 ? pk0 : pk1;
          double s1 = 0.0;
// ... 256 lines not shown
      for (int c = 0; c < NX; ++c) {
        double s2 = 0.0;
#pragma unroll
        for (int i = 0; i < NU; ++i) s2 += Gu[r * NU + i] * cs.KK[i * NX + c];
        const double inner = Gx[r * NX + c] + s2;
        Kyr[c] = dmin(dmax(cs.ys[r] * inner, -kMaxBarrierRatio), kMaxBarrierRatio);
        Ksr[c] = (-Gx[r * NX + c]) - s2;
      }
      sn[r] = affine_2r<NX>(cs.s[r], a_pr, cs.ksv[r], Ksr, dx);
      yn[r] = affine_2r<NX>(cs.y[r], a_du, cs.ky[r], Kyr, dx);
      if (sn[r] < (1.0 - tau) * cs.s[r] || yn[r] < (1.0 - tau) * cs.y[r]) feas = false;
      if (!dfinite(sn[r]) || !dfinite(yn[r])) feas = false;
    }
    }
    fail_t = (alive && !feas) ? t : fail_t;
    if (!feas) alive = false;
    st<M>(Sn + GI(t, M, 0), kLS, sn);
    st<M>(Yn + GI(t, M, 0), kLS, yn);
    if constexpr (kEarly) {
      load_step(t + 1 < N ? t + 1 : t, cs);
      PIPELINE_FENCE();
    }
    double g[M];
    Cons::template eval<NX, NU>(cc, rx, u, g);
    if constexpr (NC == 1) run_cost += Obj::running_cost(oc, xrt, t, rx, u);
    st<M>(Gn + GI(t, M, 0), kLS, g);
    double *ev = d.ev + GI((size_t)a * N + t, 2 * Cons::NSEG, 0);
#pragma unroll
    for (int c = 0; c < Cons::NSEG; ++c) {
      const int off = Cons::seg_off(c), dim = Cons::seg_dim(c);
      double n1 = 0.0, ninf = 0.0, ls = 0.0;
      for (int i = 0; i < dim; ++i) {
        const double r = g[off + i] + sn[off + i];
        n1 += l2norm ? r * r : fabs(r);
        ninf = dmax(ninf, fabs(r));
        const double ysp = yn[off + i] * sn[off + i];
        ev_icomp = dmax(ev_icomp, fabs(ysp - mu));
        ys_lo = dmin(ys_lo, ysp); ys_hi = dmax(ys_hi, ysp);
        ls += solver_log(dmax(sn[off + i], kEpsSlack));
      }
      ev_max = dmax(ev_max, ninf);
      if (c == 0 && NC == 1) ev_total0 += n1; else ev[(size_t)(Cons::NSEG + c) * kLS] = n1;
      ev[(size_t)c * kLS] = ls;
    }
  };
  StepIn ra;
  if constexpr (NC > 1) {
    static_assert(NC == 1 || kPing, "two consumers: ping-pong records with one step of look-ahead only");
    StepIn R0, R1;
    load_step(ci < N ? ci : N - 1, R0);
    prime();
    auto stop_at = [&](int tt) { return tt > __hip_atomic_load(&s_abort, __ATOMIC_RELAXED, __HIP_MEMORY_SCOPE_WORKGROUP); };
    int t = ci, last = -1;
    bool stopped = false;
    for (; t + NC < N; t += 2 * NC) {
      if (stop_at(t)) { stopped = true; break; }
      step(t, R0, R1); last = t;
      if (stop_at(t + NC)) { stopped = true; break; }
      step(t + NC, R1, R0); last = t + NC;
      if (__builtin_amdgcn_ballot_w64(alive) == 0ull) {
        __hip_atomic_fetch_min(&s_abort, last, __ATOMIC_RELAXED, __HIP_MEMORY_SCOPE_WORKGROUP);
        stopped = true; break;
      }
    }
    if (!stopped && t < N && !stop_at(t)) step(t, R0, R1);
    const bool aborted = __hip_atomic_load(&s_abort, __ATOMIC_RELAXED, __HIP_MEMORY_SCOPE_WORKGROUP) != 0x7fffffff;
    if (aborted) __hip_atomic_store(&s_consv[ci], kAbort, __ATOMIC_RELAXED, __HIP_MEMORY_SCOPE_WORKGROUP);
    if (ci == 1) {
      s_pfail[lane] = fail_t; s_palive[lane] = alive ? 1 : 0;
      s_pmax[lane] = ev_max; s_pmax[64 + lane] = ev_icomp; s_pmax[128 + lane] = ys_lo; s_pmax[192 + lane] = ys_hi;
      __builtin_amdgcn_fence(__ATOMIC_RELEASE, "workgroup");
      __hip_atomic_store(&s_done1, 1, __ATOMIC_RELAXED, __HIP_MEMORY_SCOPE_WORKGROUP);
      return;
    }
    wait_ge(&s_done1, 1);
    __builtin_amdgcn_fence(__ATOMIC_ACQUIRE, "workgroup");
    fail_t = s_pfail[lane] < fail_t ? s_pfail[lane] : fail_t;
    alive = alive && (s_palive[lane] != 0);
    ev_max = dmax(ev_max, s_pmax[lane]); ev_icomp = dmax(ev_icomp, s_pmax[64 + lane]);
    ys_lo = dmin(ys_lo, s_pmax[128 + lane]); ys_hi = dmax(ys_hi, s_pmax[192 + lane]);
    if (__hip_atomic_load(&s_abort, __ATOMIC_RELAXED, __HIP_MEMORY_SCOPE_WORKGROUP) != 0x7fffffff) {
      __hip_atomic_store(&s_consv[0], kAbort, __ATOMIC_RELAXED, __HIP_MEMORY_SCOPE_WORKGROUP);
      if (active) d.t_steps[ti] = fail_t;
      return;
    }
  } else if constexpr (kPing) {
    StepIn R[2];
#pragma unroll
    for (int j = 0; j < 1; ++j) load_step(j < N ? j : N - 1, R[j]);
    prime();
    int t = 0;
    for (; t + 1 < N; t += 2) {
#pragma unroll
      for (int j = 0; j <= 1; ++j) step(t + j, R[j], R[(j + 1) % 2]);
      if (__builtin_amdgcn_ballot_w64(alive) == 0ull) {
        __hip_atomic_store(s_cons, kAbort, __ATOMIC_RELAXED, __HIP_MEMORY_SCOPE_WORKGROUP);
        if (active) d.t_steps[ti] = fail_t;
        K4_TIME_END(1, t);
        return;
      }
    }
#pragma unroll
    for (int j = 0; j <= 1; ++j) if (t + j < N) step(t + j, R[j], R[(j + 1) % 2]);
  } else {
    if constexpr (kChunk) load_chunk(0, 0, ck0); else load_step(0, ra);
    prime();
    for (int t = 0; t < N; ++t) {
      step(t, ra, ra);
      if (__builtin_amdgcn_ballot_w64(alive) == 0ull) {
        __hip_atomic_store(s_cons, kAbort, __ATOMIC_RELAXED, __HIP_MEMORY_SCOPE_WORKGROUP);
        if (active) d.t_steps[ti] = fail_t;
        return;
      }
    }
  }
  wait_ge(&s_prod, N + kRing + 1);
  K4_TIME_END(1, N);
  if (active) d.t_steps[ti] = fail_t;
  if (alive && s_pstat[lane] <= N) alive = false;
  if (!alive) return;
  if constexpr (NC > 1) run_cost = s_prun[lane];
  const double cost_new = run_cost + s_pcost[lane];
  const double *evb = d.ev + GI((size_t)a * N, 2 * Cons::NSEG, 0);
  const size_t tstride = (size_t)d.NB * (2 * Cons::NSEG) * kLS;
  if constexpr (NC > 1) {
    const double *q = evb + (size_t)Cons::NSEG * kLS;
    int t = 0;
    for (; t + 3 < N; t += 4) {
      const double v0 = q[(size_t)t * tstride], v1 = q[(size_t)(t + 1) * tstride], v2 = q[(size_t)(t + 2) * tstride], v3 = q[(size_t)(t + 3) * tstride];
      ev_total0 += v0; ev_total0 += v1; ev_total0 += v2; ev_total0 += v3;
    }
    for (; t < N; ++t) ev_total0 += q[(size_t)t * tstride];
  }
  double total = ev_total0, mer = cost_new;
  for (int c = 1; c < Cons::NSEG; ++c) {
    const double *q = evb + (size_t)(Cons::NSEG + c) * kLS;
    int t = 0;
    for (; t + 3 < N; t += 4) {
      const double v0 = q[(size_t)t * tstride], v1 = q[(size_t)(t + 1) * tstride], v2 = q[(size_t)(t + 2) * tstride], v3 = q[(size_t)(t + 3) * tstride];
      total += v0; total += v1; total += v2; total += v3;
    }
    for (; t < N; ++t) total += q[(size_t)t * tstride];
  }
  for (int c = 0; c < Cons::NSEG; ++c) {
    const double *q = evb + (size_t)c * kLS;
    int t = 0;
    for (; t + 3 < N; t += 4) {
      const double v0 = q[(size_t)t * tstride], v1 = q[(size_t)(t + 1) * tstride], v2 = q[(size_t)(t + 2) * tstride], v3 = q[(size_t)(t + 3) * tstride];
      mer -= mu * v0; mer -= mu * v1; mer -= mu * v2; mer -= mu * v3;
    }
    for (; t < N; ++t) mer -= mu * q[(size_t)t * tstride];
  }
  if constexpr (TERM) {
    double n1 = 0.0, ninf = 0.0, dp = 0.0;
    for (int c = 0; c < P->n_term; ++c) {
      const TermDev &td = P->terms[c];
      if (td.kind != CDDP_HIP_TERM_EQUALITY) continue;
      for (int r = 0; r < td.dim; ++r) {
        const double h = s_xN[r * 64 + lane] - P->pool[td.off_target + r];
        n1 += l2norm ? h * h : fabs(h);
        ninf = dmax(ninf, fabs(h));
      }
    }
    total += n1; ev_max = dmax(ev_max, ninf);
    for (int c = 0; c < P->n_term; ++c) {
      const TermDev &td = P->terms[c];
      if (td.kind != CDDP_HIP_TERM_EQUALITY) continue;
      for (int r = 0; r < td.dim; ++r) {
        const int j = td.offset + r;
        const double h = s_xN[r * 64 + lane] - P->pool[td.off_target + r];
        const double lam = d.LamT[(size_t)j * d.Bp + b] + a_pr * d.dLamT[(size_t)j * d.Bp + b];
        if (!dfinite(lam)) return;
        d.LamTt[((size_t)a * kPTMax + j) * d.Bp + b] = lam;
        dp += lam * h;
      }
    }
    mer += dp;
  }
  const double th = l2norm ? sqrt(total) : total;
  const double theta_new = dmax(th, ev_max), phi_new = mer, ipr = ev_max, icomp = ev_icomp;
  if (!dfinite(phi_new) || !dfinite(theta_new) || !dfinite(ipr) || !dfinite(icomp)) return;
  bool accept = false;
  {
    const double expected_improvement = a_pr * d.dV0[b];
    const int fn = d.filt_n[b];
    const double cv_old = (fn == 0) ? 0.0 : d.filt[(size_t)(kFilterCap + fn - 1) * d.Bp + b];
    const double high_ref = (fn == 0) ? d.filter_theta[b] : cv_old;
    const double merit_old = d.merit[b];
    if (theta_new > o.filter_max_violation_threshold) {
      if (theta_new < (1 - o.filter_violation_acceptance_threshold) * high_ref) accept = true;
    } else if (dmax(theta_new, cv_old) < o.filter_min_violation_for_armijo_check && expected_improvement < 0) {
      if (phi_new < merit_old + o.filter_armijo_constant * expected_improvement) accept = true;
    } else {
      if (phi_new < merit_old - o.filter_merit_acceptance_threshold * theta_new ||
          theta_new < (1 - o.filter_violation_acceptance_threshold) * cv_old) accept = true;
    }
  }
  d.t_cost[ti] = cost_new; d.t_merit[ti] = phi_new; d.t_theta[ti] = theta_new;
  d.t_inf_pr[ti] = ipr; d.t_inf_comp[ti] = icomp;
  d.t_ysmin[ti] = ys_lo; d.t_ysmax[ti] = ys_hi;
  d.t_success[ti] = accept ? 1 : 0;
}

#undef GI
}
```

cddp-cpp_amd/csrc/knobs.hpp:

```cpp
#pragma once
#include <climits>
#include <cstdlib>
#include <cstring>
#include <string>

namespace cddp_dev {

inline char env_first(const char *name) { const char *e = std::getenv(name); return e ? e[0] : 0; }
inline bool env_is(const char *name, const char *v) { const char *e = std::getenv(name); return e && !std::strcmp(e, v); }
inline int env_num(const char *name, int dflt, int lo, int hi) { const char *e = std::getenv(name); const int n = e ? std::atoi(e) : dflt; return (n >= lo && n <= hi) ? n : dflt; }
inline long env_long(const char *name, long dflt) { const char *e = std::getenv(name); return e ? std::atol(e) : dflt; }
inline std::string env_str(const char *name) { const char *e = std::getenv(name); return e ? e : ""; }

struct Knobs {
  enum Sweep { kSweepCoop, kSweepLane, kSweepElem, kSweepMfma };
  int sweep = env_is("CDDP_HIP_SWEEP", "lane") ? kSweepLane : env_is("CDDP_HIP_SWEEP", "elem") ? kSweepElem : env_is("CDDP_HIP_SWEEP", "mfma") ? kSweepMfma : kSweepCoop;
  bool t4 = env_first("CDDP_HIP_T4") != '0';
  int sweep_roles = env_num("CDDP_HIP_SWEEP_ROLES", 1, 0, 2);
  bool coop_h2 = env_first("CDDP_HIP_COOP_H") == '2';
  bool coop_w1 = env_first("CDDP_HIP_COOP_W") == '1';
  int k4_na = env_num("CDDP_HIP_K4_NA", 1, 1, 3);
  bool k4_consumers2 = env_first("CDDP_HIP_K4_CONSUMERS") == '2';
  bool ms_lane_rollout = env_is("CDDP_HIP_MS_ROLLOUT", "lane");
  bool lg_lane_rollout = env_is("CDDP_HIP_LG_ROLLOUT", "lane");
  bool graph = env_first("CDDP_HIP_GRAPH") == '1';
  char ls_stages = env_first("CDDP_HIP_LS_STAGES");
  int ls_first = env_num("CDDP_HIP_LS_FIRST", 0, INT_MIN, INT_MAX);
  long ls_two_max_waves = env_long("CDDP_HIP_LS_TWO_MAX_WAVES", 768);
  int ls_small_frac = env_num("CDDP_HIP_LS_SMALL_FRAC", 3, 1, INT_MAX);
  int ls_margin = env_num("CDDP_HIP_LS_MARGIN", 1, 0, 8);
  int run_ahead = env_num("CDDP_HIP_RUNAHEAD", 1, 0, 16);
  int poll_every = env_num("CDDP_HIP_POLL_EVERY", 4, 1, INT_MAX);
  bool event_fence = env_first("CDDP_HIP_EVENT_FENCE") == '1';
  bool debug_ladder = std::getenv("CDDP_HIP_DEBUG_LADDER") != nullptr;
  int groups = env_num("CDDP_HIP_GROUPS", 0, INT_MIN, INT_MAX);
  bool chunking = env_num("CDDP_HIP_CHUNK", 1, INT_MIN, INT_MAX) > 0;
  int chunk = env_num("CDDP_HIP_CHUNK", 0, 1, INT_MAX);
  int partition = env_num("CDDP_HIP_PARTITION", 0, 1, 16);
  bool cumask_set = std::getenv("CDDP_HIP_CUMASK") != nullptr;
  std::string cumask = env_str("CDDP_HIP_CUMASK");
  bool pingpong = env_first("CDDP_HIP_PINGPONG") == '1';
  bool xcd_map = env_first("CDDP_HIP_XCD_MAP") != '0';
  int fail_costate = env_num("CDDP_HIP_TEST_FAIL_COSTATE", 0, INT_MIN, INT_MAX);
  enum Costate { kCostateAuto, kCostateSync, kCostateShadow };
  int costate = env_is("CDDP_HIP_COSTATE", "sync") ? kCostateSync : env_is("CDDP_HIP_COSTATE", "shadow") ? kCostateShadow : kCostateAuto;
  int fail_shadow = env_num("CDDP_HIP_TEST_FAIL_SHADOW", 0, 1, INT_MAX);
};

}
```

cddp-cpp_amd/csrc/launch.hpp:

```cpp
#pragma once
#include <algorithm>
#include <vector>
#include "knobs.hpp"
#include "kernels_te.hpp"
#include "kernels_pcm.hpp"
#include "kernels_elem.hpp"
#include "kernels_mfma.hpp"
#include "kernels_logddp.hpp"
#include "kernels_msipddp.hpp"

namespace cddp_dev {

struct SweepHop { hipStream_t s; hipEvent_t ev_in, ev_out; };
inline thread_local const SweepHop *tl_sweep_hop = nullptr;
inline thread_local hipError_t tl_order_error = hipSuccess;
inline void order_check(hipError_t e) { if (e != hipSuccess && tl_order_error == hipSuccess) tl_order_error = e; }
inline hipStream_t sweep_hop_in(hipStream_t s) {
  const SweepHop *h = tl_sweep_hop;
  if (!h || h->s == s) return s;
  order_check(hipEventRecord(h->ev_in, s));
  order_check(hipStreamWaitEvent(h->s, h->ev_in, 0));
  return h->s;
}
inline void sweep_hop_out(hipStream_t s) {
  const SweepHop *h = tl_sweep_hop;
  if (!h || h->s == s) return;
  order_check(hipEventRecord(h->ev_out, h->s));
  order_check(hipStreamWaitEvent(s, h->ev_out, 0));
}

struct Route {
  enum Sweep { kCoop, kLane, kElem, kMfma, kRowSplit, kOneWave };
  enum Rollout { kPair, kGroup2, kGroup3, kTwoConsumers, kLaneRollout };
  int sweep = kCoop;
  int roles_nh = 0;
  bool ms_split = false;
  int rollout = kPair;
  int t4 = 0;
};

struct KernelSet {
  int model, nx, nu, m;
  int cst_size;
  int te_rec_size, te_group;
  const char *name;
  bool (*matches)(const ProblemDev &);
  Route (*route)(const DevBuf &, int solver, const Knobs &);
  void (*derivs)(const DevBuf &, const Route &, int force, hipStream_t);
  void (*backward)(const DevBuf &, const Route &, int solver, int force, int count_iter, hipStream_t);
  void (*forward)(const DevBuf &, const Route &, int solver, int a0, int na, int phase_req, int force, int first_only, hipStream_t);
  void (*costate)(const DevBuf &, const Route &, int solver, int a0, int na, int phase_req, int force, int first_only, hipStream_t);
  void (*update)(const DevBuf &, const Route &, int stage, int n1, int is_last, int do_count, hipStream_t);
  void (*init)(const DevBuf &, int mode, hipStream_t);
  void (*stage)(const DevBuf &, int copy_xu, int ipddp, hipStream_t);
  int (*sweep_blocks)(const DevBuf &);
  int (*shadow_extra)(const DevBuf &, const Route &);
  void (*shadow_flush)(const DevBuf &, const DevBuf *, hipStream_t);
  bool logddp_ddp;
  bool has_msipddp;
  bool has_logddp;
  int ms_cst_size;
};

template <class Model, class Cons> struct PcTwoConsumers { static constexpr bool value = false; };
template <class Cons> struct PcTwoConsumers<UnicycleModel, Cons> {
  static constexpr int kRec = 5 * Cons::M + UnicycleModel::NU * UnicycleModel::NX + (Cons::HAS_X ? UnicycleModel::NX : 1) + (Cons::NEEDS_U ? UnicycleModel::NU : 1);
  static constexpr bool value = Cons::M >= 4 && kRec > 16 && kRec <= 40;
};

template <class Model, class Cons, bool TERM = false>
struct Launcher {
  static bool matches(const ProblemDev &P) {
    return P.model == Model::ID && P.nx == Model::NX && P.nu == Model::NU && Cons::matches(P) && (TERM ? P.n_term > 0 : P.n_term == 0);
  }
  static constexpr bool kLean = !TERM && Cons::M > 0;
  static constexpr int cst_size() { if constexpr (kLean) return CstLayout<Model, Cons>::SIZE; else return 0; }
  static constexpr bool kTeCoop = TERM && !Cons::HAS_X;
  static constexpr int te_rec_size() { if constexpr (kTeCoop) return TeCfg<Model, Cons>::REC; else return 0; }
  static constexpr int kLogMaxNx = 16;
  static constexpr bool kLog = !TERM && Model::NX <= kLogMaxNx;
  static constexpr int kMsMaxNx = 13;
  static constexpr bool kMs = !TERM && Model::NX <= kMsMaxNx && (Cons::M == 0 || Model::NU == 1 || Model::NX == Model::NU);
  static constexpr int ms_cst_size() { if constexpr (kMs && Cons::M > 0) return MsCst<Model, Cons>::SIZE; else return 0; }
  static dim3 gridB(const DevBuf &d) { return dim3((d.B + 63) / 64); }
  template <int RB> static constexpr bool roles_fit() {
    if constexpr (!kLean || Model::NX > 8) return false;
    else return (size_t)RoleCfg<Model, Cons, RB>::RING * 8 + (size_t)CoopCfg<Model>::TPW * CoopCfg<Model>::STRIDE * 8 <= (size_t)72 * 1024;
  }
  static constexpr bool kRoles = roles_fit<2>();
  static Route route(const DevBuf &d, int solver, const Knobs &k) {
    Route r;
    const bool lane = k.sweep == Knobs::kSweepLane || (d.ddp && solver != CDDP_HIP_SOLVER_CLDDP);
    r.sweep = lane ? Route::kLane : Route::kCoop;
    r.ms_split = d.ms && d.cst && !lane;
    if (solver == CDDP_HIP_SOLVER_IPDDP && !lane) {
      if constexpr (kLean && Model::NX > 8) {
        if (Model::NX <= 15 && Model::NU <= 8 && k.sweep == Knobs::kSweepMfma) r.sweep = Route::kMfma;
        else if (k.coop_h2) r.sweep = Route::kRowSplit;
        else if (Cons::HAS_X || k.coop_w1) r.sweep = Route::kOneWave;
      } else if constexpr (kLean) {
        if (Model::NX <= 4 && Model::NU <= 2 && k.sweep == Knobs::kSweepElem) r.sweep = Route::kElem;
        else if (kRoles && d.cst && !d.ms && !d.lg && k.sweep != Knobs::kSweepElem) r.roles_nh = k.sweep_roles;
      } else if constexpr (TERM) {
        if (!(kTeCoop && d.te_cst)) r.sweep = Route::kLane;
      }
    }
    if (solver == CDDP_HIP_SOLVER_LOGDDP) r.rollout = k.lg_lane_rollout ? Route::kLaneRollout : Route::kPair;
    if (solver == CDDP_HIP_SOLVER_MSIPDDP) r.rollout = k.ms_lane_rollout ? Route::kLaneRollout : Route::kPair;
    if constexpr (kLean) {
      if (solver == CDDP_HIP_SOLVER_IPDDP) {
        if (PcmTraits<Model, Cons>::kOk && k.k4_na >= 2) r.rollout = k.k4_na == 3 ? Route::kGroup3 : Route::kGroup2;
        else if (PcTwoConsumers<Model, Cons>::value && k.k4_consumers2) r.rollout = Route::kTwoConsumers;
      }
    }
    if constexpr (CoopCfg<Model>::G == 16) {
      if (k.t4 && k.sweep != Knobs::kSweepLane && k.sweep != Knobs::kSweepMfma && !d.ddp) {
        if constexpr (kLean) r.t4 = (d.cst && !d.ms && !d.lg) ? 1 : 0;
        else if constexpr (kTeCoop) r.t4 = d.te_cst ? 1 : 0;
      }
    }
    return r;
  }
  static void derivs(const DevBuf &d, const Route &r, int force, hipStream_t s) {
    if constexpr (kLean) {
      if (d.cst && !d.ms && !d.lg) {
        if (r.roles_nh > 0) return;
        if constexpr (Model::NX <= 8) {
          hipLaunchKernelGGL((k_condense<Model, Cons, true>), dim3((d.B + 63) / 64, d.N), dim3(64), 0, s, d, d.P, d.xref_traj, force);
          return;
        } else {
          hipLaunchKernelGGL((k_derivs<Model>), dim3((d.B + 63) / 64, d.N), dim3(64), 0, s, d, d.P, d.xref_traj, force);
          hipLaunchKernelGGL((k_condense<Model, Cons, false>), dim3((d.B + 63) / 64, d.N), dim3(64), 0, s, d, d.P, d.xref_traj, force);
          return;
// ... 30 lines not shown
            hipLaunchKernelGGL((k_ms_post<Model, Cons>), gridW, dim3(64), 0, s, d, d.P, force);
            return;
          }
        }
        hipLaunchKernelGGL((k_backward_msipddp<Model, Cons>), gridB(d), dim3(64), 0, s, d, d.P, d.xref_traj, force, count_iter);
      }
      return;
    }
    const bool lane_sweep = r.sweep == Route::kLane;
    const dim3 gridC(coop_grid<CoopCfg<Model>::TPW>(d.B, d.xcd_map));
    if (solver == CDDP_HIP_SOLVER_CLDDP) {
      if (lane_sweep)
        hipLaunchKernelGGL((k_backward_clddp<Model>), gridB(d), dim3(64), 0, s, d, d.P, d.xref_traj, force, count_iter);
      else {
        hipLaunchKernelGGL((k_backward_coop_plain<Model, true>), gridC, dim3(64), 0, sweep_hop_in(s), d, d.P, d.xref_traj, force, count_iter);
        sweep_hop_out(s);
      }
    } else if constexpr (kLean) {
      if (lane_sweep)
        hipLaunchKernelGGL((k_backward_ipddp_lean<Model, Cons>), gridB(d), dim3(64), 0, s, d, d.P, d.xref_traj, force, count_iter);
      else if constexpr (Model::NX > 8) {
        if (r.sweep == Route::kMfma) {
          if constexpr (Model::NX <= 15 && Model::NU <= 8) {
            const dim3 gridW(((d.NB + 7) / 8) * 8 * 64);
            hipLaunchKernelGGL((k_backward_ipddp_mfma<Model, Cons>), gridW, dim3(64), 0, s, d, d.P, d.xref_traj, force, count_iter);
            hipLaunchKernelGGL((k_dx_rollout_wave<Model>), gridW, dim3(64), 0, s, d, force);
          }
        } else if (r.sweep == Route::kRowSplit) {
          hipLaunchKernelGGL((k_backward_ipddp_coop_big<Model, Cons, 2>), dim3(coop_grid<CoopCfg<Model>::TPW / 2>(d.B, d.xcd_map)), dim3(64), 0, s, d, d.P, d.xref_traj, force, count_iter);
        } else {
          if constexpr (!Cons::HAS_X) {
            if (r.sweep != Route::kOneWave) hipLaunchKernelGGL((k_backward_ipddp_coop_big2<Model, Cons>), gridC, dim3(128), 0, sweep_hop_in(s), d, d.P, d.xref_traj, force, count_iter);
          }
          if (r.sweep == Route::kOneWave) hipLaunchKernelGGL((k_backward_ipddp_coop_big<Model, Cons, 1>), gridC, dim3(64), 0, sweep_hop_in(s), d, d.P, d.xref_traj, force, count_iter);
          sweep_hop_out(s);
        }
      }
      else {
        if (r.sweep == Route::kElem) {
          if constexpr (Model::NX <= 4 && Model::NU <= 2)
            hipLaunchKernelGGL((k_backward_ipddp_elem<Model, Cons>), dim3(coop_grid<4>(d.B, d.xcd_map)), dim3(64), 0, s, d, d.P, d.xref_traj, force, count_iter);
        } else if (r.roles_nh > 0) {
          if constexpr (kRoles) {
            const hipStream_t ss = sweep_hop_in(s);
            const dim3 gridC(coop_grid<CoopCfg<Model>::TPW>(d.B, d.xcd_map) + (unsigned)(d.cs_extra > 0 ? d.cs_extra : 0));
            if (r.roles_nh == 1) {
              if constexpr (roles_fit<3>()) hipLaunchKernelGGL((k_backward_ipddp_coop<Model, Cons, 1, 3>), gridC, dim3(128), 0, ss, d, d.P, d.xref_traj, force, count_iter);
              else hipLaunchKernelGGL((k_backward_ipddp_coop<Model, Cons, 1, 2>), gridC, dim3(128), 0, ss, d, d.P, d.xref_traj, force, count_iter);
            } else {
              if constexpr (roles_fit<4>()) hipLaunchKernelGGL((k_backward_ipddp_coop<Model, Cons, 2, 4>), gridC, dim3(192), 0, ss, d, d.P, d.xref_traj, force, count_iter);
              else if constexpr (roles_fit<3>()) hipLaunchKernelGGL((k_backward_ipddp_coop<Model, Cons, 2, 3>), gridC, dim3(192), 0, ss, d, d.P, d.xref_traj, force, count_iter);
              else hipLaunchKernelGGL((k_backward_ipddp_coop<Model, Cons, 2, 2>), gridC, dim3(192), 0, ss, d, d.P, d.xref_traj, force, count_iter);
            }
            sweep_hop_out(s);
          }
        } else {
          hipLaunchKernelGGL((k_backward_ipddp_coop<Model, Cons>), gridC, dim3(64), 0, sweep_hop_in(s), d, d.P, d.xref_traj, force, count_iter);
          sweep_hop_out(s);
        }
      }
      if constexpr (kRoles) { if (r.roles_nh > 0) return; }
      hipLaunchKernelGGL((k_post<Model, Cons>), dim3((d.B + 63) / 64, d.N), dim3(64), 0, s, d, d.P, force);
    } else if constexpr (!TERM && Cons::M == 0) {
      if (lane_sweep)
        hipLaunchKernelGGL((k_backward_ipddp<Model, Cons, TERM>), gridB(d), dim3(64), 0, s, d, d.P, d.xref_traj, force, count_iter);
      else {
        hipLaunchKernelGGL((k_backward_coop_plain<Model, false>), gridC, dim3(64), 0, sweep_hop_in(s), d, d.P, d.xref_traj, force, count_iter);
        sweep_hop_out(s);
      }
    } else {
      if constexpr (kTeCoop) {
        if (r.sweep == Route::kCoop) {
          hipLaunchKernelGGL((k_backward_te_coop<Model, Cons>), gridC, dim3(64), 0, sweep_hop_in(s), d, d.P, d.xref_traj, force, count_iter);
          sweep_hop_out(s);
          const int tiles = (d.B + 63) / 64;
          int tstep = (int)(((long long)tiles * d.N) / 1024); if (tstep < 1) tstep = 1; if (tstep > 16) tstep = 16;
          hipLaunchKernelGGL((k_te_post<Model, Cons>), dim3(tiles, (d.N + tstep - 1) / tstep), dim3(64), 0, s, d, d.P, force, tstep);
          return;
        }
      }
      hipLaunchKernelGGL((k_backward_ipddp<Model, Cons, TERM>), gridB(d), dim3(64), 0, s, d, d.P, d.xref_traj, force, count_iter);
    }
  }
  static void forward(const DevBuf &d, const Route &r, int solver, int a0, int na, int phase_req, int force, int first_only, hipStream_t s) {
    if (na <= 0) return;
    const dim3 grid((d.B + 63) / 64, na);
    if (solver == CDDP_HIP_SOLVER_LOGDDP) {
      if constexpr (kLog) {
        if (r.rollout == Route::kLaneRollout) hipLaunchKernelGGL((k_forward_logddp<Model, Cons>), grid, dim3(64), 0, s, d, d.P, d.xref_traj, a0, 0, phase_req, force);
        else hipLaunchKernelGGL((k_forward_logddp_pc<Model, Cons>), grid, dim3(128), 0, s, d, d.P, d.xref_traj, a0, phase_req, force);
      }
      return;
    }
    if (solver == CDDP_HIP_SOLVER_MSIPDDP) {
      if constexpr (kMs) {
        if (r.rollout == Route::kLaneRollout || !d.ladder_sorted) hipLaunchKernelGGL((k_forward_msipddp<Model, Cons>), grid, dim3(64), 0, s, d, d.P, d.xref_traj, a0, 0, phase_req, force);
        else hipLaunchKernelGGL((k_forward_msipddp_pc<Model, Cons>), grid, dim3(128), 0, s, d, d.P, d.xref_traj, a0, phase_req, force);
      }
      return;
    }
    if (solver == CDDP_HIP_SOLVER_CLDDP)
      hipLaunchKernelGGL((k_forward_clddp<Model>), grid, dim3(64), 0, s, d, d.P, d.xref_traj, a0, 0, phase_req, force);
    else
    {
      if constexpr (kLean) {
        if constexpr (PcmTraits<Model, Cons>::kOk) {
          if (r.rollout == Route::kGroup3) { hipLaunchKernelGGL((k_forward_ipddp_pcm<Model, Cons, 3>), dim3((d.B + 63) / 64, (na + 2) / 3), dim3(256), 0, s, d, d.P, d.xref_traj, a0, na, phase_req, force); return; }
          if (r.rollout == Route::kGroup2) { hipLaunchKernelGGL((k_forward_ipddp_pcm<Model, Cons, 2>), dim3((d.B + 63) / 64, (na + 1) / 2), dim3(192), 0, s, d, d.P, d.xref_traj, a0, na, phase_req, force); return; }
        }
        if constexpr (PcTwoConsumers<Model, Cons>::value) {
          if (r.rollout == Route::kTwoConsumers) { hipLaunchKernelGGL((k_forward_ipddp_pc<Model, Cons, false, 2>), grid, dim3(192), 0, s, d, d.P, d.xref_traj, a0, phase_req, force); return; }
        }
        hipLaunchKernelGGL((k_forward_ipddp_pc<Model, Cons>), grid, dim3(128), 0, s, d, d.P, d.xref_traj, a0, phase_req, force);
      } else {
        if constexpr (kTeCoop && Cons::M > 0) {
          if (r.sweep == Route::kCoop) {
            hipLaunchKernelGGL((k_forward_ipddp_pc<Model, Cons, true>), grid, dim3(128), 0, s, d, d.P, d.xref_traj, a0, phase_req, force);
            return;
          }
        }
        hipLaunchKernelGGL((k_forward_ipddp<Model, Cons, TERM>), grid, dim3(64), 0, s, d, d.P, d.xref_traj, a0, 0, phase_req, force);
      }
    }
    (void)first_only;
  }
  static void costate(const DevBuf &d, const Route &r, int solver, int a0, int na, int phase_req, int force, int first_only, hipStream_t s) {
    if (solver == CDDP_HIP_SOLVER_MSIPDDP) {
      if constexpr (kMs) {
        if (na <= 0 || r.rollout == Route::kLaneRollout || !d.ladder_sorted) return;
        if (!force && first_only == 2) hipLaunchKernelGGL((k_pick_candidate<0>), dim3((d.B + 63) / 64), dim3(64), 0, s, d, a0, na, phase_req, force);
        hipLaunchKernelGGL((k_rows_msipddp<Model, Cons>), dim3((d.B + 63) / 64, d.N), dim3(64), 0, s, d, d.P, a0, na, phase_req, force, first_only);
      }
      return;
    }
    if (na <= 0 || solver == CDDP_HIP_SOLVER_CLDDP || solver == CDDP_HIP_SOLVER_LOGDDP) return;
    if (!force && first_only == 2) hipLaunchKernelGGL((k_pick_candidate<0>), dim3((d.B + 63) / 64), dim3(64), 0, s, d, a0, na, phase_req, force);
    if constexpr (Model::NX > 8) {
      if (!force && first_only != 0) {
        hipLaunchKernelGGL((k_costate_one<Model>), dim3((d.B + 63) / 64, d.N + 1), dim3(64), 0, s, d, a0, na, phase_req, first_only);
        return;
      }
    }
    hipLaunchKernelGGL((k_costate<Model>), dim3((d.B + 63) / 64, d.N + 1), dim3(64), 0, s, d, a0, na, phase_req, force, force ? 0 : first_only);
  }
  static int shadow_extra(const DevBuf &d, const Route &r) {
    if constexpr (kRoles) {
      if (r.roles_nh <= 0) return 0;
      const int items = d.NB * (d.N + 1), per = 4 * (1 + r.roles_nh);
      const int own = (int)coop_grid<CoopCfg<Model>::TPW>(d.B, d.xcd_map);
      return std::max(1, std::min((items + per - 1) / per, 2 * own));
    }
    return 0;
  }
  static int sweep_blocks(const DevBuf &d) { return (int)coop_grid<CoopCfg<Model>::TPW>(d.B, d.xcd_map); }
  static void shadow_flush(const DevBuf &d, const DevBuf *dm, hipStream_t s) {
    if constexpr (kRoles) {
      const dim3 grid((d.B + 63) / 64, d.N + 1);
      if (d.cs_want > 0) hipLaunchKernelGGL((k_costate_flush<Model>), grid, dim3(64), 0, s, d);
      if (!dm) return;
      hipLaunchKernelGGL((k_value_merge<Model::NX>), grid, dim3(64), 0, s, *dm);
    }
  }
  static void update(const DevBuf &d, const Route &r, int stage, int n1, int is_last, int do_count, hipStream_t s) {
    if (d.lg) {
      if constexpr (kLog) hipLaunchKernelGGL((k_update_logddp<Model, Cons>), gridB(d), dim3(64), 0, s, d, d.P, stage, n1, is_last, do_count);
      return;
    }
    if (d.ms) {
      if constexpr (kMs) hipLaunchKernelGGL((k_update_msipddp<Model, Cons>), gridB(d), dim3(64), 0, s, d, d.P, stage, n1, is_last, do_count);
      return;
    }
    DevBuf dd = d;
    if constexpr (kTeCoop && Cons::M > 0) dd.ev_valid = r.sweep == Route::kCoop ? 1 : 0;
    hipLaunchKernelGGL((k_update<Model, Cons, TERM>), gridB(d), dim3(64), 0, s, dd, d.P, d.xref_traj, stage, n1, is_last, do_count);
  }
  static void init(const DevBuf &d, int mode, hipStream_t s) {
    if (d.lg) {
      if constexpr (kLog) hipLaunchKernelGGL((k_init_logddp<Model, Cons>), gridB(d), dim3(64), 0, s, d, d.P, d.xref_traj, mode);
      return;
    }
    if (d.ms) {
      if constexpr (kMs) hipLaunchKernelGGL((k_init_msipddp<Model, Cons>), gridB(d), dim3(64), 0, s, d, d.P, d.xref_traj, mode);
      return;
    }
    hipLaunchKernelGGL((k_init<Model, Cons, TERM>), gridB(d), dim3(64), 0, s, d, d.P, d.xref_traj, mode);
  }
  static void stage(const DevBuf &d, int copy_xu, int ipddp, hipStream_t s) {
    hipLaunchKernelGGL((k_stage<Model, Cons>), dim3((d.B + 63) / 64, d.N + 1), dim3(64), 0, s, d, copy_xu, ipddp);
  }
  static KernelSet set(const char *name) {
    KernelSet k;
    k.model = Model::ID; k.nx = Model::NX; k.nu = Model::NU; k.m = Cons::M; k.name = name; k.cst_size = cst_size(); k.te_rec_size = te_rec_size(); k.te_group = CoopCfg<Model>::G;
    k.matches = &matches; k.route = &route; k.derivs = &derivs; k.backward = &backward; k.forward = &forward;
    k.costate = &costate; k.update = &update; k.init = &init; k.stage = &stage; k.shadow_extra = &shadow_extra; k.sweep_blocks = &sweep_blocks; k.shadow_flush = &shadow_flush; k.has_logddp = kLog; k.logddp_ddp = Model::kHasHess; k.has_msipddp = kMs; k.ms_cst_size = ms_cst_size();
    return k;
  }
};

void register_pendulum(std::vector<KernelSet> &);
void register_cartpole(std::vector<KernelSet> &);
// ... 15 lines not shown
```

cddp-cpp_amd/pyapi.py:

```python
import ctypes as C
import os
import numpy as np

_HERE = os.path.dirname(os.path.abspath(__file__))
REPO = os.path.dirname(_HERE)
HIP_LIB_PATH = os.environ.get("CDDP_HIP_LIB") or os.path.join(_HERE, "lib", "libcddp_hip.so")

ABI_VERSION = 5
MAX_MODEL_PARAMS = 24
NAME_LEN = 48

MODEL_PENDULUM, MODEL_CARTPOLE, MODEL_UNICYCLE, MODEL_LTI = 0, 1, 2, 3
MODEL_QUADROTOR, MODEL_MANIPULATOR, MODEL_QUADROTOR_EULER12, MODEL_MANIPULATOR7 = 4, 5, 6, 7
MODEL_BICYCLE, MODEL_CAR, MODEL_HCW = 8, 9, 10
MODEL_EULER_ATTITUDE, MODEL_QUATERNION_ATTITUDE, MODEL_MRP_ATTITUDE = 11, 12, 13
MODEL_SPACECRAFT_TWOBODY, MODEL_SPACECRAFT_LANDING2D = 14, 15
MODEL_DUBINS_CAR, MODEL_DREYFUS_ROCKET, MODEL_ACROBOT, MODEL_USV_3DOF, MODEL_FORKLIFT = 16, 17, 18, 19, 20
MODEL_QUADROTOR_RATE, MODEL_SPACECRAFT_LINEAR_FUEL, MODEL_SPACECRAFT_NONLINEAR = 21, 22, 23
EULER, HEUN, RK3, RK4 = 0, 1, 2, 3
SOLVER_CLDDP, SOLVER_IPDDP, SOLVER_LOGDDP, SOLVER_MSIPDDP = 0, 1, 2, 3
CON_CONTROL_BOX, CON_STATE_BOX, CON_BALL, CON_LINEAR = 0, 1, 2, 3
CON_SOC, CON_THRUST, CON_MAX_THRUST = 4, 5, 6
TERM_EQUALITY, TERM_INEQUALITY = 0, 1
STATUS_RUNNING, STATUS_OPTIMAL, STATUS_ACCEPTABLE, STATUS_MAX_ITERATIONS, STATUS_REG_LIMIT, STATUS_MAX_CPU_TIME, STATUS_REG_LIMIT_CONVERGED = range(7)
# ... 640 lines not shown
                np.diag([100.0] * 6 + [0.0] * 4), np.array([0.0] * 6 + [1.0, 0.0, 0.0, 1.0]), model_params=[1.0, 1.0, 1.0, 1.0], options=o)
    if constrained:
        p.add_control_box("ControlConstraint", -0.3 * np.ones(3), 0.3 * np.ones(3))
    p.x0 = np.array([0.02, -0.01, 0.01, 0.0, 0.01, 0.0, 1.0, 0.0, 0.0, 1.0])
    return p


def batch_x0(problem, batch, seed, spread=None):
    rng = np.random.default_rng(seed)
    x0 = np.tile(problem.x0, (batch, 1)).astype(np.float64)
    if spread is None:
        spread = 0.1 * np.ones(problem.nx)
    pert = rng.uniform(-1.0, 1.0, size=(batch, problem.nx)) * np.asarray(spread)[None, :]
    pert[0] = 0.0
    return np.ascontiguousarray(x0 + pert)


def batch_U0(problem, batch):
    if hasattr(problem, "U0_const"):
        return np.ascontiguousarray(np.tile(problem.U0_const, (batch, problem.N, 1)).astype(np.float64))
    return None


_hip_libs = {}


def default_trig():
    return "libm" if (os.environ.get("CDDP_HIP_LIB") and os.environ.get("CDDP_HIP_TRIG") == "libm") else "shared"


def load_hip(trig=None):
    trig = trig or default_trig()
    if trig not in ("shared", "libm"):
        raise ValueError("trig must be None, 'shared' or 'libm'")
    if "lib" not in _hip_libs:
        path = HIP_LIB_PATH
        if not os.path.exists(path):
            raise RuntimeError("HIP library missing: %s -- run __graft_entry__.build(); "
                               "the product has no CPU fallback" % path)
        lib = C.CDLL(path)
        lib.cddp_hip_last_error.restype = C.c_char_p
        lib.cddp_hip_status_string.restype = C.c_char_p
        lib.cddp_hip_create.argtypes = [C.POINTER(ProblemStruct), C.c_int, C.c_int, C.POINTER(C.c_void_p)]
        lib.cddp_hip_mpc_advance.argtypes = MPC_ADVANCE_ARGTYPES; lib.cddp_hip_mpc_advance.restype = C.c_int
        lib.cddp_hip_mpc_run.argtypes = MPC_RUN_ARGTYPES; lib.cddp_hip_mpc_run.restype = C.c_int
        for name, at in list(PLANT_ARGTYPES.items()) + list(DEVICE_IO_ARGTYPES.items()):
            fn = getattr(lib, name); fn.argtypes = at; fn.restype = C.c_int
        _hip_libs["lib"] = lib
    lib = _hip_libs["lib"]
    if (trig == "shared") != bool(lib.cddp_hip_trig_shared()):
        raise RuntimeError("trig=%r asked for, but %s was built %s -DCDDP_TRIG_SHARED" %
                           (trig, HIP_LIB_PATH, "with" if lib.cddp_hip_trig_shared() else "without"))
    return lib


MPC_ADVANCE_ARGTYPES = [C.c_void_p, C.c_int, C.c_int, C.c_void_p]
MPC_RUN_ARGTYPES = [C.c_void_p, C.c_int, C.c_int, C.c_int, _dp, _dp, C.POINTER(C.c_int32), C.POINTER(C.c_int32), C.POINTER(Stats)]
PLANT_ARGTYPES = {
    "cddp_hip_plant_create": [C.POINTER(PlantDesc), C.c_int, C.c_int, C.POINTER(C.c_void_p)],
    "cddp_hip_plant_destroy": [C.c_void_p],
    "cddp_hip_plant_step": [C.c_void_p, C.c_int, C.c_void_p, C.c_void_p, C.c_void_p, C.c_void_p],
    "cddp_hip_mpc_run_plant": [C.c_void_p, C.c_void_p, C.c_int, C.c_int, C.c_int, _dp, _dp, _dp, C.POINTER(C.c_int32), C.POINTER(C.c_int32), C.POINTER(Stats)],
    "cddp_hip_track_plan": [C.c_void_p, C.c_void_p, _dp, _dp, _dp, _dp],
}
DEVICE_IO_ARGTYPES = {
    "cddp_hip_field_shape": [C.c_void_p, C.c_int, C.POINTER(C.c_int32), C.POINTER(C.c_int32)],
    "cddp_hip_get_field_device": [C.c_void_p, C.c_int, C.c_void_p],
    "cddp_hip_get_results_device": [C.c_void_p, C.c_void_p, C.c_void_p],
    "cddp_hip_set_initial_device": [C.c_void_p, C.c_void_p, C.c_void_p, C.c_void_p],
    "cddp_hip_get_live_slots": [C.c_void_p, C.POINTER(C.c_int32), C.POINTER(C.c_int32)],
}

EXPORTED_SYMBOLS = [
    "cddp_hip_default_options", "cddp_hip_abi_version", "cddp_hip_trig_shared", "cddp_hip_last_error", "cddp_hip_device_count",
    "cddp_hip_status_string", "cddp_hip_build_alphas", "cddp_hip_create", "cddp_hip_destroy",
    "cddp_hip_set_stream", "cddp_hip_set_initial", "cddp_hip_initialize", "cddp_hip_backward",
    "cddp_hip_forward", "cddp_hip_solve", "cddp_hip_get_results", "cddp_hip_get_trajectory",
    "cddp_hip_get_gains", "cddp_hip_get_value", "cddp_hip_get_linearization", "cddp_hip_get_duals", "cddp_hip_get_costates", "cddp_hip_get_backward_scalars",
    "cddp_hip_get_history", "cddp_hip_get_terminal", "cddp_hip_write_gather_records_device", "cddp_hip_dual_dim", "cddp_hip_batch",
    "cddp_hip_set_timing_detail", "cddp_hip_history_capacity", "cddp_hip_set_barrier_state", "cddp_hip_num_groups", "cddp_hip_concurrency", "cddp_hip_comm_unique_id", "cddp_hip_comm_init", "cddp_hip_comm_destroy", "cddp_hip_comm_info", "cddp_hip_get_plan_head", "cddp_hip_allgather_results",
    "cddp_hip_backward_stacks", "cddp_hip_stacks_create_abi", "cddp_hip_stacks_destroy", "cddp_hip_set_stacks", "cddp_hip_set_defect_stack", "cddp_hip_set_control_box", "cddp_hip_set_hessian_stacks", "cddp_hip_set_constraint_stacks",
    "cddp_hip_stacks_backward", "cddp_hip_stacks_last_kernel_ms", "cddp_hip_stacks_last_sweep_form", "cddp_hip_stacks_factor_cache", "cddp_hip_stacks_get_gains", "cddp_hip_stacks_get_constraint_gains",
    "cddp_hip_stacks_get_scalars", "cddp_hip_set_terminal_equality", "cddp_hip_stacks_get_terminal", "cddp_hip_plugin_solve", "cddp_hip_plugin_solve_terminal", "cddp_hip_plugin_set_host_threads", "cddp_hip_plugin_last_stats", "cddp_hip_model_eval", "cddp_hip_set_options", "cddp_hip_set_initial_state", "cddp_hip_forget_solver_state", "cddp_hip_set_duals", "cddp_hip_set_terminal",
    "cddp_hip_costate_mode", "cddp_hip_costate_redos", "cddp_hip_mpc_advance", "cddp_hip_mpc_run",
    "cddp_hip_plant_create", "cddp_hip_plant_destroy", "cddp_hip_plant_step", "cddp_hip_mpc_run_plant", "cddp_hip_track_plan",
    "cddp_hip_field_shape", "cddp_hip_get_field_device", "cddp_hip_get_results_device", "cddp_hip_set_initial_device", "cddp_hip_get_live_slots",
]


class HipError(RuntimeError):
    pass


class HipBatchSolver:

    def __init__(self, problem, batch, device=0, trig=None):
        self.lib = load_hip(trig)
        self.p = problem; self.B = batch
        self.h = C.c_void_p()
        rc = self.lib.cddp_hip_create(C.byref(problem.c), batch, device, C.byref(self.h))
        self._check(rc)
        self.m = self.lib.cddp_hip_dual_dim(self.h)
        self._user_stream = False; self._device = int(device)

    def _check(self, rc):
        if rc != 0:
            raise HipError("cddp_hip error %d: %s" % (rc, self.lib.cddp_hip_last_error().decode()))

    def close(self):
        if self.h:
            self.lib.cddp_hip_destroy(self.h); self.h = C.c_void_p()

    def __del__(self):
        try:
            self.close()
        except Exception:
            pass

    def num_groups(self):
        return int(self.lib.cddp_hip_num_groups(self.h))

    def concurrency(self):
        return int(self.lib.cddp_hip_concurrency(self.h))

    def costate_mode(self):
        return int(self.lib.cddp_hip_costate_mode(self.h))

    def costate_redos(self):
        return int(self.lib.cddp_hip_costate_redos(self.h))

    def set_stream(self, stream_ptr):
        self._check(self.lib.cddp_hip_set_stream(self.h, C.c_void_p(stream_ptr)))
        self._user_stream = True

    def set_timing_detail(self, detail):
        self._check(self.lib.cddp_hip_set_timing_detail(self.h, int(detail)))

    def set_initial(self, x0, U0=None, X0=None):
        x0 = _arr(x0); assert x0.shape == (self.B, self.p.nx)
        U0 = _arr(U0) if U0 is not None else None; X0 = _arr(X0) if X0 is not None else None
        self._check(self.lib.cddp_hip_set_initial(self.h, _ptr(x0), _ptr(U0), _ptr(X0)))

    def initialize(self):
        self._check(self.lib.cddp_hip_initialize(self.h))

    def set_options(self, options):
        self._check(self.lib.cddp_hip_set_options(self.h, C.byref(options)))

    def set_warm_start(self, flag=True):
        self.p.options.warm_start = 1 if flag else 0
        self.set_options(self.p.options)

    def set_initial_state(self, x0):
        x0 = _arr(x0).reshape(self.B, self.p.nx)
        self._check(self.lib.cddp_hip_set_initial_state(self.h, _ptr(x0)))

    def forget_solver_state(self):
        self._check(self.lib.cddp_hip_forget_solver_state(self.h))

    def set_duals(self, S=None, Y=None):
        S = _arr(S) if S is not None else None; Y = _arr(Y) if Y is not None else None
        self._check(self.lib.cddp_hip_set_duals(self.h, _ptr(S), _ptr(Y)))

    def set_barrier_state(self, mu=None, reg=None):
        mu = _arr(mu).reshape(self.B) if mu is not None else None
        reg = _arr(reg).reshape(self.B) if reg is not None else None
        self._check(self.lib.cddp_hip_set_barrier_state(self.h, _ptr(mu), _ptr(reg)))

    def set_terminal_state(self, S_T=None, Y_T=None, Lambda_T=None):
        a = [(_arr(v) if v is not None else None) for v in (S_T, Y_T, Lambda_T)]
        self._check(self.lib.cddp_hip_set_terminal(self.h, _ptr(a[0]), _ptr(a[1]), _ptr(a[2])))

    def backward(self):
        ok = np.zeros(self.B, dtype=np.int32)
        self._check(self.lib.cddp_hip_backward(self.h, ok.ctypes.data_as(C.POINTER(C.c_int32))))
        return ok

    def forward(self, alphas):
        a = _arr(alphas); t = np.zeros((self.B, a.size), dtype=TRIAL_DTYPE)
        self._check(self.lib.cddp_hip_forward(self.h, _ptr(a), a.size, t.ctypes.data_as(C.c_void_p)))
        return t

    def solve(self):
        st = Stats()
        self._check(self.lib.cddp_hip_solve(self.h, C.byref(st)))
        return st

    def results(self):
        r = np.zeros(self.B, dtype=RESULT_DTYPE)
        self._check(self.lib.cddp_hip_get_results(self.h, r.ctypes.data_as(C.c_void_p)))
        return r

    def trajectory(self):
        X = np.zeros((self.B, self.p.N + 1, self.p.nx)); U = np.zeros((self.B, self.p.N, self.p.nu))
        self._check(self.lib.cddp_hip_get_trajectory(self.h, _ptr(X), _ptr(U)))
        return X, U

    def plan_head(self):
        u0 = np.zeros((self.B, self.p.nu)); x1 = np.zeros((self.B, self.p.nx))
        self._check(self.lib.cddp_hip_get_plan_head(self.h, _ptr(u0), _ptr(x1)))
        return u0, x1

    def mpc_advance(self, mode, x_next=None, shift_duals=False):
        flags = MPC_SHIFT_DUALS if shift_duals else 0
        keep = None
        if x_next is None:
            ptr = None
        elif isinstance(x_next, np.ndarray) or not hasattr(x_next, "data_ptr"):
            keep = _arr(x_next).reshape(self.B, self.p.nx); ptr = keep.ctypes.data
        else:
            import torch
            if not x_next.is_cuda or x_next.dtype != torch.float64 or tuple(x_next.shape) != (self.B, self.p.nx):
# ... 561 lines not shown
```

include/cddp_hip.h:

```cpp
#ifndef CDDP_HIP_H
#define CDDP_HIP_H

#include <stdint.h>

#ifdef __cplusplus
extern "C" {
#endif

#define CDDP_HIP_ABI_VERSION 5
#define CDDP_HIP_MAX_MODEL_PARAMS 24
#define CDDP_HIP_NAME_LEN 48
#define CDDP_HIP_MAX_ALPHAS 32


enum cddp_hip_model {
  CDDP_HIP_MODEL_PENDULUM = 0,
  CDDP_HIP_MODEL_CARTPOLE = 1,
  CDDP_HIP_MODEL_UNICYCLE = 2,
  CDDP_HIP_MODEL_LTI = 3,
  CDDP_HIP_MODEL_QUADROTOR = 4,
  CDDP_HIP_MODEL_MANIPULATOR = 5,
  CDDP_HIP_MODEL_QUADROTOR_EULER12 = 6,
  CDDP_HIP_MODEL_MANIPULATOR7 = 7,
  CDDP_HIP_MODEL_BICYCLE = 8,
// ... 180 lines not shown
  int32_t iterations;
  int32_t status;
  int32_t n_backward;
  int32_t n_forward;
} cddp_hip_result;

typedef struct cddp_hip_gather_record {
  double final_objective;
  int32_t iterations;
  int32_t status;
} cddp_hip_gather_record;

typedef struct cddp_hip_trial {
  double alpha, alpha_pr, alpha_du;
  double cost, merit_function, theta, inf_pr, inf_comp;
  int32_t success;
  int32_t _pad;
} cddp_hip_trial;

typedef struct cddp_hip_stats {
  double solve_ms;
  double backward_ms;
  double forward_ms;
  double update_ms;
  int64_t sweeps;
  int64_t rollouts;
  int64_t rollouts_launched;
  int64_t traj_iterations;
  int32_t outer_iterations;
  int32_t n_converged;
  int32_t kernel_launches;
  int32_t timing_detail;
  int64_t rollout_steps;
} cddp_hip_stats;

enum {
  CDDP_HIP_TIMING_ROLLOUT = 0,
  CDDP_HIP_TIMING_ALL = 1,
  CDDP_HIP_TIMING_SWEEP = 2
};

typedef struct cddp_hip_handle cddp_hip_handle;


int cddp_hip_abi_version(void);
int cddp_hip_trig_shared(void);
const char *cddp_hip_last_error(void);
int cddp_hip_device_count(void);
const char *cddp_hip_status_string(int status);

int cddp_hip_build_alphas(const cddp_hip_options *opt, double *alphas, int cap);

int cddp_hip_create(const cddp_hip_problem *problem, int batch, int device,
                    cddp_hip_handle **out);
int cddp_hip_destroy(cddp_hip_handle *h);

int cddp_hip_set_stream(cddp_hip_handle *h, void *hip_stream);

int cddp_hip_set_timing_detail(cddp_hip_handle *h, int detail);

int cddp_hip_set_initial(cddp_hip_handle *h, const double *x0, const double *U0,
                         const double *X0);

int cddp_hip_initialize(cddp_hip_handle *h);

int cddp_hip_set_options(cddp_hip_handle *h, const cddp_hip_options *options);

int cddp_hip_set_initial_state(cddp_hip_handle *h, const double *x0);

int cddp_hip_forget_solver_state(cddp_hip_handle *h);

int cddp_hip_set_duals(cddp_hip_handle *h, const double *S, const double *Y);
int cddp_hip_set_terminal(cddp_hip_handle *h, const double *S_T, const double *Y_T, const double *Lambda_T);
int cddp_hip_set_barrier_state(cddp_hip_handle *h, const double *mu, const double *reg);

int cddp_hip_backward(cddp_hip_handle *h, int32_t *ok);

int cddp_hip_forward(cddp_hip_handle *h, const double *alphas, int n_alphas,
                     cddp_hip_trial *trials);

int cddp_hip_solve(cddp_hip_handle *h, cddp_hip_stats *stats);
int cddp_hip_costate_mode(cddp_hip_handle *h);
int cddp_hip_costate_redos(cddp_hip_handle *h);

enum cddp_hip_mpc_mode {
  CDDP_HIP_MPC_KEEP_PLAN = 0,
  CDDP_HIP_MPC_SHIFT_EXISTING = 1,
  CDDP_HIP_MPC_SHIFT_PROVIDED = 2
};
enum { CDDP_HIP_MPC_SHIFT_DUALS = 1,
       CDDP_HIP_MPC_X_DEVICE   = 2 };
int cddp_hip_mpc_advance(cddp_hip_handle *h, int mode, int flags, const double *x_next );
int cddp_hip_mpc_run(cddp_hip_handle *h, int steps, int mode, int flags,
                     double *U_applied , double *X_visited ,
                     int32_t *iterations , int32_t *status , cddp_hip_stats *stats_sum);

typedef struct cddp_hip_plant_desc {
  int32_t abi_version;
  int32_t model, integrator;
  int32_t substeps;
  int32_t nx, nu;
  int32_t params_per_trajectory;
  int32_t _pad;
  double dt;
  const double *model_params;
  const double *lti_A, *lti_B;
  const double *u_lower, *u_upper;
} cddp_hip_plant_desc;
typedef struct cddp_hip_plant cddp_hip_plant;
enum { CDDP_HIP_PLANT_DEVICE = 1 };

int cddp_hip_plant_create(const cddp_hip_plant_desc *desc, int batch, int device, cddp_hip_plant **out);
int cddp_hip_plant_destroy(cddp_hip_plant *p);
int cddp_hip_plant_step(cddp_hip_plant *p, int flags, const double *x , const double *u ,
                        const double *w , double *x_next );
int cddp_hip_mpc_run_plant(cddp_hip_handle *h, cddp_hip_plant *plant, int steps, int mode, int flags,
                           const double *W ,
                           double *U_applied, double *X_visited, int32_t *iterations, int32_t *status, cddp_hip_stats *stats_sum);
int cddp_hip_track_plan(cddp_hip_handle *h, cddp_hip_plant *plant, const double *x0 ,
                        const double *W , double *X_out , double *U_out );

int cddp_hip_get_results(cddp_hip_handle *h, cddp_hip_result *results );
int cddp_hip_get_plan_head(cddp_hip_handle *h, double *u0, double *x1);
int cddp_hip_get_trajectory(cddp_hip_handle *h, double *X , double *U );
int cddp_hip_get_gains(cddp_hip_handle *h, double *K, double *k);
int cddp_hip_get_value(cddp_hip_handle *h, double *Vx, double *Vxx);
int cddp_hip_get_linearization(cddp_hip_handle *h, double *A , double *Bm );
int cddp_hip_get_duals(cddp_hip_handle *h, double *S, double *Y, double *G);
int cddp_hip_get_costates(cddp_hip_handle *h, double *Lambda, int32_t *rows);
int cddp_hip_get_terminal(cddp_hip_handle *h, double *S_T, double *Y_T, double *G_T, double *Lambda_T, int32_t *dims);
int cddp_hip_get_backward_scalars(cddp_hip_handle *h, double *dV, double *reg);
int cddp_hip_get_history(cddp_hip_handle *h, int hist_batch, double *hist, int32_t *counts);
int cddp_hip_history_capacity(cddp_hip_handle *h);

int cddp_hip_write_gather_records_device(cddp_hip_handle *h, void *device_ptr);

enum cddp_hip_field { CDDP_HIP_FIELD_X = 0, CDDP_HIP_FIELD_U, CDDP_HIP_FIELD_K, CDDP_HIP_FIELD_KFF,
                      CDDP_HIP_FIELD_VX, CDDP_HIP_FIELD_VXX, CDDP_HIP_FIELD_A, CDDP_HIP_FIELD_B,
                      CDDP_HIP_FIELD_S, CDDP_HIP_FIELD_Y, CDDP_HIP_FIELD_G, CDDP_HIP_FIELD_LAMBDA };
int cddp_hip_field_shape(cddp_hip_handle *h, int field, int32_t *rows, int32_t *cols);
int cddp_hip_get_field_device(cddp_hip_handle *h, int field, double *out_dev);
int cddp_hip_get_results_device(cddp_hip_handle *h, double *cols_dev , int32_t *icols_dev );
int cddp_hip_set_initial_device(cddp_hip_handle *h, const double *x0_dev, const double *U0_dev, const double *X0_dev);
int cddp_hip_get_live_slots(cddp_hip_handle *h, int32_t *slots, int32_t *n_slots);

#define CDDP_HIP_COMM_ID_BYTES 128
int cddp_hip_comm_unique_id(char *id_out );
int cddp_hip_comm_init(const char *id_in, int world, int rank, int device, void **comm_out);
int cddp_hip_comm_destroy(void *comm);
int cddp_hip_comm_info(void *comm, int *count_out, int *rank_out);
int cddp_hip_allgather_results(cddp_hip_handle *h, void *comm , int world, int shard_capacity,
                               void *recv_device);

int cddp_hip_dual_dim(cddp_hip_handle *h);
int cddp_hip_batch(cddp_hip_handle *h);
int cddp_hip_num_groups(cddp_hip_handle *h);
int cddp_hip_concurrency(cddp_hip_handle *h);

typedef struct cddp_hip_stack_handle cddp_hip_stack_handle;
enum cddp_hip_stacks_branch {
  CDDP_HIP_STACKS_CLDDP = 0,
  CDDP_HIP_STACKS_IPDDP = 1,
  CDDP_HIP_STACKS_IPDDP_PATH = 2,
  CDDP_HIP_STACKS_MSIPDDP = 4,
  CDDP_HIP_STACKS_MSIPDDP_PATH = 5,
  CDDP_HIP_STACKS_IPDDP_TERM_EQ = 6,
// ... 77 lines not shown
```

Before: 106,400.

## Fuse two-stage line search into one launch with in-kernel success-mask polling

```diff
diff --git a/cddp-cpp_amd/csrc/capi.hip b/cddp-cpp_amd/csrc/capi.hip
--- a/cddp-cpp_amd/csrc/capi.hip
+++ b/cddp-cpp_amd/csrc/capi.hip
@@ -185,6 +185,8 @@
   std::map<unsigned long long, hipGraphExec_t> graphs;
   bool shadow_bufs = false;
   int cs_epoch = 0;
+  unsigned long long *h_ls = nullptr;
+  long long ls_counts[3] = {0, 0, 0};
   int n_redo = 0;
   bool last_shadow = false;
   bool ever_solved = false;
@@ -639,7 +641,7 @@
   }
   DA(d.n_active, 1);
   DA(d.win_hist, CDDP_HIP_MAX_ALPHAS + 1);
-  DA(h->d_launched, 1);
+  DA(h->d_launched, ls_words(Bp / 64));
   DA(h->dP, 1);
   DA(h->d_Xinit, d.planeX); DA(h->d_Uinit, d.planeU);
   if (problem->x_ref_traj) {
@@ -680,6 +682,7 @@
   if (h->ev_poll) hipEventDestroy(h->ev_poll);
   if (h->ev_poll2) hipEventDestroy(h->ev_poll2);
   if (h->h_poll) hipHostFree(h->h_poll);
+  if (h->h_ls) hipHostFree(h->h_ls);
   if (h->h_bad) hipHostFree(h->h_bad);
   if (h->d_head) hipFree(h->d_head);
   if (h->h_head) hipHostFree(h->h_head);
@@ -908,7 +911,7 @@
   HIPCHK(hipMemcpyAsync(h->dP, &tmp, sizeof(ProblemDev), hipMemcpyHostToDevice, h->stream));
   DevBuf dcall = h->d;
   dcall.ladder_sorted = ladder_strictly_decreasing(tmp.alphas, h->d.n_alphas);
-  h->ks->forward(dcall, h->route, h->P.solver, 0, n_alphas, PH_FWD1, 1, 0, h->stream);
+  h->ks->forward(dcall, h->route, h->P.solver, 0, n_alphas, PH_FWD1, 1, 0, h->stream, 0, 0);
   h->ks->costate(dcall, h->route, h->P.solver, 0, n_alphas, PH_FWD1, 1, 0, h->stream);
   HIPCHK(hipGetLastError());
   const DevBuf &d = h->d;
@@ -946,6 +949,8 @@
   bool two_stage_marks = false, first_rule = true, pinned = false, one_stage = true, done = false, cpu_time_hit = false, use_graph = false;
   int k1 = 1, k_cap = 1, k_cap2 = 1;
   bool shadow = false, force_sync = false, pre_has_state = false, redo_needed = false;
+  bool inkernel = false;
+  int poll_us = kLsPollUs;
   int stamp0 = 0;
   long waves_all = 0, per_alpha_waves = 1, two_stage_max_waves = 768;
   std::vector<int> hist_now, hist_prev;
@@ -1033,11 +1038,16 @@
     poll_evs[0] = h->ev_poll; poll_evs[1] = h->ev_poll2;
     win_enq = win_dig = 0; ran_ahead = false;
     if (!h->h_poll) HIPCHK(hipHostMalloc((void **)&h->h_poll, sizeof(int) * 2 * kPollWords));
-    HIPCHK(hipMemsetAsync(h->d_launched, 0, sizeof(unsigned long long), s));
+    HIPCHK(hipMemsetAsync(h->d_launched, 0, sizeof(unsigned long long) * kLsGran, s));
     HIPCHK(hipEventRecord(h->ev_begin, s));
     pre_has_state = h->has_state;
     shadow = !force_sync && shadow_eligible(h, conc) && max_it > 0;
     redo_needed = false;
+    inkernel = shadow && P.ls_rule == CDDP_HIP_LS_FIRST_SUCCESS && h->knob->ls_inkernel &&
+               (h->route.rollout == Route::kPair || h->route.rollout == Route::kTwoConsumers);
+    poll_us = h->knob->ls_poll_us >= 0 ? h->knob->ls_poll_us : kLsPollUs;
+    h->ls_counts[0] = h->ls_counts[1] = h->ls_counts[2] = 0;
+    if (inkernel && !h->h_ls) HIPCHK(hipHostMalloc((void **)&h->h_ls, sizeof(unsigned long long) * kLsGran));
     h->last_shadow = shadow; h->ever_solved = true;
     if (shadow) HIPCHK(hipMemsetAsync(h->d.cs_bad, 0, sizeof(int), s));
     stamp0 = h->cs_epoch;
@@ -1084,7 +1094,8 @@
     hipStream_t sf = h->cu.fwd ? h->cu.fwd : s;
     auto to_fwd = [&](int k) { if (sf != s) { order_check(hipEventRecord(h->cu.ev[k], s)); order_check(hipStreamWaitEvent(sf, h->cu.ev[k], 0)); } };
     auto from_fwd = [&](int k) { if (sf != s) { order_check(hipEventRecord(h->cu.ev[k], sf)); order_check(hipStreamWaitEvent(s, h->cu.ev[k], 0)); } };
-    two_stage_marks = !one_stage;
+    const bool split = !one_stage && inkernel;
+    two_stage_marks = !one_stage && !split;
     mark(0);
     ks->derivs(d, r, 0, s);
     tl_sweep_hop = h->cu.sweep ? &h->cu.hop : nullptr;
@@ -1094,8 +1105,8 @@
     mark(1);
     to_fwd(0);
     if (fwd_wait) hipStreamWaitEvent(sf, fwd_wait, 0);
-    if (one_stage) {
-      ks->forward(d, r, P.solver, 0, na, PH_FWD1, 0, first_rule ? 1 : 0, sf);
+    if (one_stage || split) {
+      ks->forward(d, r, P.solver, 0, na, PH_FWD1, 0, first_rule ? 1 : 0, sf, split ? k1 : 0, poll_us);
       if (fwd_done) hipEventRecord(fwd_done, sf);
       from_fwd(1);
       mark(2);
@@ -1104,7 +1115,7 @@
       mark(3);
       launches += shadow ? 3 : 4;
     } else {
-      ks->forward(d, r, P.solver, 0, k1, PH_FWD1, 0, 1, sf);
+      ks->forward(d, r, P.solver, 0, k1, PH_FWD1, 0, 1, sf, 0, 0);
       from_fwd(1);
       mark(2);
       if (!shadow) ks->costate(d, r, P.solver, 0, k1, PH_FWD1, 0, 1, s);
@@ -1118,7 +1129,7 @@
       ks->update(d, r, 1, k1, last, 0, s);
       mark(3);
       to_fwd(2);
-      ks->forward(d, r, P.solver, k1, na - k1, PH_FWD2, 0, 1, sf);
+      ks->forward(d, r, P.solver, k1, na - k1, PH_FWD2, 0, 1, sf, 0, 0);
       if (fwd_done) hipEventRecord(fwd_done, sf);
       from_fwd(3);
       mark(4);
@@ -1220,8 +1231,10 @@
     const DevBuf &d = h->d;
     hipStream_t s = h->stream;
     HIPCHK(hipEventRecord(h->ev_end, s));
+    if (inkernel) HIPCHK(hipMemcpyAsync(h->h_ls, h->d_launched, sizeof(unsigned long long) * kLsGran, hipMemcpyDeviceToHost, s));
     HIPCHK(hipStreamSynchronize(s));
     HIPCHK(hipGetLastError());
+    if (inkernel) { h->ls_counts[0] = (long long)h->h_ls[kLsRan]; h->ls_counts[1] = (long long)h->h_ls[kLsRet]; h->ls_counts[2] = (long long)h->h_ls[kLsGiveUp]; }
     if (shadow && *h->h_bad != 0) { redo_needed = true; return 0; }
     if (tl_order_error != hipSuccess) {
       const hipError_t oe = tl_order_error; tl_order_error = hipSuccess;
@@ -1668,6 +1681,12 @@
   int n = 0;
   for (Inner *q : h->g) n += q->n_redo;
   return n;
+}
+int cddp_hip_ls_stage_counts(cddp_hip_handle *h, long long *counts) {
+  if (!h || !counts) return -1;
+  counts[0] = counts[1] = counts[2] = 0;
+  for (Inner *q : h->g) for (int i = 0; i < 3; ++i) counts[i] += q->ls_counts[i];
+  return 0;
 }
 int cddp_hip_concurrency(cddp_hip_handle *h) { return h ? std::max(1, std::min(h->conc, (int)h->g.size())) : -1; }
 
diff --git a/cddp-cpp_amd/csrc/dev_types.hpp b/cddp-cpp_amd/csrc/dev_types.hpp
--- a/cddp-cpp_amd/csrc/dev_types.hpp
+++ b/cddp-cpp_amd/csrc/dev_types.hpp
@@ -42,6 +42,11 @@
 constexpr int kLS = 64;
 
 constexpr int kSinkDoubles = 1024 * 64;
+
+constexpr int kLsRan = 1, kLsRet = 2, kLsGiveUp = 3, kLsGran = 8;
+constexpr unsigned kLsTag = 0x4c533231u;
+constexpr size_t ls_words(int NB) { return (size_t)kLsGran + (size_t)NB * CDDP_HIP_MAX_ALPHAS * 2; }
+constexpr int kLsPollUs = 10000;
 
 struct DevBuf {
   int B, Bp, N, n_slots, n_alphas, hist_batch, hist_cap, NB;
diff --git a/cddp-cpp_amd/csrc/kernels_coop.hpp b/cddp-cpp_amd/csrc/kernels_coop.hpp
--- a/cddp-cpp_amd/csrc/kernels_coop.hpp
+++ b/cddp-cpp_amd/csrc/kernels_coop.hpp
@@ -204,6 +204,11 @@
       return;
     }
     if (blockIdx.x == 0 && threadIdx.x == 0 && !force) *d.n_active = 0;
+    {
+      const int own = (int)gridDim.x - (d.cs_extra > 0 ? d.cs_extra : 0), ng = d.NB * CDDP_HIP_MAX_ALPHAS * 2;
+      for (int i = (int)blockIdx.x * (int)blockDim.x + (int)threadIdx.x; i < ng; i += own * (int)blockDim.x)
+        __hip_atomic_store(d.launched + kLsGran + i, 0ull, __ATOMIC_RELAXED, __HIP_MEMORY_SCOPE_AGENT);
+    }
     const bool act = (b < d.B) && (force || d.phase[b] == PH_ACTIVE);
     if (__builtin_amdgcn_ballot_w64(act) == 0ull) return;
     if (threadIdx.x == 0) {
diff --git a/cddp-cpp_amd/csrc/kernels_lean.hpp b/cddp-cpp_amd/csrc/kernels_lean.hpp
--- a/cddp-cpp_amd/csrc/kernels_lean.hpp
+++ b/cddp-cpp_amd/csrc/kernels_lean.hpp
@@ -638,7 +638,7 @@
 
 template <class Model, class Cons, bool TERM = false, int NC = 1>
 __global__ __launch_bounds__(64 * (1 + NC)) void k_forward_ipddp_pc(DevBuf d, const ProblemDev *__restrict__ Pk, const double *__restrict__ xrt,
-                                                                    int a0, int phase_req, int force) {
+                                                                    int a0, int phase_req, int force, int k1, int poll_us) {
   constexpr int NX = Model::NX, NU = Model::NU, M = Cons::M;
   typedef Objective<NX, NU> Obj;
   static_assert(M > 0, "two-role rollout is for path-constrained problems");
@@ -654,6 +654,7 @@
   [[maybe_unused]] __shared__ int s_pfail[kL2], s_palive[kL2];
   [[maybe_unused]] __shared__ double s_pmax[4 * kL2];
   [[maybe_unused]] __shared__ double s_prun[kL2];
+  __shared__ unsigned s_need[2];
   __shared__ int s_pstat[64];
   __shared__ double s_pcost[64];
   __shared__ double s_xN[TERM ? NX * 64 : 1];
@@ -669,11 +670,51 @@
   const ProblemDev *__restrict__ P = Pk;
   const cddp_hip_options &o = P->opt;
   const int N = d.N;
-  const bool active = (b < d.B) && (force || d.phase[b] == phase_req);
+  bool active = (b < d.B) && (force || d.phase[b] == phase_req);
   if (__builtin_amdgcn_ballot_w64(active) == 0ull) return;
   if (producer) { s_pstat[lane] = N + 2; if (lane == 0) { s_prod = 0; s_consv[0] = 0; s_consv[1] = 0; if constexpr (NC > 1) { s_abort = 0x7fffffff; s_done1 = 0; } } }
   Obj::stage(P, s_obj, (int)threadIdx.x, 64 * (1 + NC));
+  const bool stage2 = k1 > 0 && a >= k1;
+  if (stage2 && producer) {
+    const unsigned long long *gran = d.launched + kLsGran + (size_t)blockIdx.x * (CDDP_HIP_MAX_ALPHAS * 2);
+    const unsigned long long in_phase = __builtin_amdgcn_ballot_w64(active);
+    const bool mine = lane < 2 * k1;
+    const unsigned long long t0 = wall_clock64(), bound = (unsigned long long)poll_us * 100ull;
+    unsigned long long v = 0ull;
+    bool gave_up = false;
+    for (;;) {
+      if (wall_clock64() - t0 >= bound) { gave_up = true; break; }
+      if (mine) v = __hip_atomic_load(gran + lane, __ATOMIC_RELAXED, __HIP_MEMORY_SCOPE_AGENT);
+      if (__builtin_amdgcn_ballot_w64(mine && (unsigned)(v >> 32) != kLsTag) == 0ull) break;
+      __builtin_amdgcn_s_sleep(16);
+    }
+    unsigned lo = 0u, hi = 0u;
+    if (!gave_up)
+      for (int i = 0; i < k1; ++i) {
+        lo |= (unsigned)__builtin_amdgcn_readlane((int)(unsigned)v, 2 * i);
+        hi |= (unsigned)__builtin_amdgcn_readlane((int)(unsigned)v, 2 * i + 1);
+      }
+    const unsigned long long need = in_phase & ~(((unsigned long long)hi << 32) | lo);
+    if (lane == 0) {
+      s_need[0] = (unsigned)need; s_need[1] = (unsigned)(need >> 32);
+      atomicAdd(d.launched + (need != 0ull ? kLsRan : kLsRet), 1ull);
+      if (gave_up) atomicAdd(d.launched + kLsGiveUp, 1ull);
+    }
+  }
   __syncthreads();
+  if (stage2) {
+    const unsigned n0 = __builtin_amdgcn_readfirstlane(s_need[0]), n1 = __builtin_amdgcn_readfirstlane(s_need[1]);
+    if ((n0 | n1) == 0u) return;
+    active = active && ((((lane < 32 ? n0 : n1) >> (lane & 31)) & 1u) != 0u);
+  }
+  auto publish_mask = [&](const bool ok) {
+    if (k1 > 0 && a < k1) {
+      const unsigned long long m = __builtin_amdgcn_ballot_w64(ok);
+      if (lane < 2)
+        __hip_atomic_store(d.launched + kLsGran + ((size_t)blockIdx.x * CDDP_HIP_MAX_ALPHAS + a) * 2 + lane,
+                           ((unsigned long long)kLsTag << 32) | (unsigned long long)(unsigned)(m >> (32 * lane)), __ATOMIC_RELAXED, __HIP_MEMORY_SCOPE_AGENT);
+    }
+  };
   const int bb = (b < d.B) ? b : 0;
   const int cur = (b < d.B) ? d.cur[b] : 0;
   const int slot = trial_slot(cur, a);
@@ -1096,6 +1137,7 @@
     if (__hip_atomic_load(&s_abort, __ATOMIC_RELAXED, __HIP_MEMORY_SCOPE_WORKGROUP) != 0x7fffffff) {
       __hip_atomic_store(&s_consv[0], kAbort, __ATOMIC_RELAXED, __HIP_MEMORY_SCOPE_WORKGROUP);
       if (active) d.t_steps[ti] = fail_t;
+      publish_mask(false);
       return;
     }
   } else if constexpr (kPing) {
@@ -1111,6 +1153,7 @@
         __hip_atomic_store(s_cons, kAbort, __ATOMIC_RELAXED, __HIP_MEMORY_SCOPE_WORKGROUP);
         if (active) d.t_steps[ti] = fail_t;
         K4_TIME_END(1, t);
+        publish_mask(false);
         return;
       }
     }
@@ -1124,6 +1167,7 @@
       if (__builtin_amdgcn_ballot_w64(alive) == 0ull) {
         __hip_atomic_store(s_cons, kAbort, __ATOMIC_RELAXED, __HIP_MEMORY_SCOPE_WORKGROUP);
         if (active) d.t_steps[ti] = fail_t;
+        publish_mask(false);
         return;
       }
     }
@@ -1132,6 +1176,8 @@
   K4_TIME_END(1, N);
   if (active) d.t_steps[ti] = fail_t;
   if (alive && s_pstat[lane] <= N) alive = false;
+  bool flagged = false;
+  [&]() {
   if (!alive) return;
   if constexpr (NC > 1) run_cost = s_prun[lane];
   const double cost_new = run_cost + s_pcost[lane];
@@ -1214,6 +1260,9 @@
   d.t_inf_pr[ti] = ipr; d.t_inf_comp[ti] = icomp;
   d.t_ysmin[ti] = ys_lo; d.t_ysmax[ti] = ys_hi;
   d.t_success[ti] = accept ? 1 : 0;
+  flagged = accept;
+  }();
+  publish_mask(flagged);
 }
 
 #undef GI
diff --git a/cddp-cpp_amd/csrc/knobs.hpp b/cddp-cpp_amd/csrc/knobs.hpp
--- a/cddp-cpp_amd/csrc/knobs.hpp
+++ b/cddp-cpp_amd/csrc/knobs.hpp
@@ -29,6 +29,8 @@
   long ls_two_max_waves = env_long("CDDP_HIP_LS_TWO_MAX_WAVES", 768);
   int ls_small_frac = env_num("CDDP_HIP_LS_SMALL_FRAC", 3, 1, INT_MAX);
   int ls_margin = env_num("CDDP_HIP_LS_MARGIN", 1, 0, 8);
+  bool ls_inkernel = env_first("CDDP_HIP_LS_INKERNEL") != '0';
+  int ls_poll_us = env_num("CDDP_HIP_TEST_LS_POLL_US", -1, 0, INT_MAX);
   int run_ahead = env_num("CDDP_HIP_RUNAHEAD", 1, 0, 16);
   int poll_every = env_num("CDDP_HIP_POLL_EVERY", 4, 1, INT_MAX);
   bool event_fence = env_first("CDDP_HIP_EVENT_FENCE") == '1';
diff --git a/cddp-cpp_amd/csrc/launch.hpp b/cddp-cpp_amd/csrc/launch.hpp
--- a/cddp-cpp_amd/csrc/launch.hpp
+++ b/cddp-cpp_amd/csrc/launch.hpp
@@ -48,7 +48,7 @@
   Route (*route)(const DevBuf &, int solver, const Knobs &);
   void (*derivs)(const DevBuf &, const Route &, int force, hipStream_t);
   void (*backward)(const DevBuf &, const Route &, int solver, int force, int count_iter, hipStream_t);
-  void (*forward)(const DevBuf &, const Route &, int solver, int a0, int na, int phase_req, int force, int first_only, hipStream_t);
+  void (*forward)(const DevBuf &, const Route &, int solver, int a0, int na, int phase_req, int force, int first_only, hipStream_t, int k1, int poll_us);
   void (*costate)(const DevBuf &, const Route &, int solver, int a0, int na, int phase_req, int force, int first_only, hipStream_t);
   void (*update)(const DevBuf &, const Route &, int stage, int n1, int is_last, int do_count, hipStream_t);
   void (*init)(const DevBuf &, int mode, hipStream_t);
@@ -245,7 +245,7 @@
       hipLaunchKernelGGL((k_backward_ipddp<Model, Cons, TERM>), gridB(d), dim3(64), 0, s, d, d.P, d.xref_traj, force, count_iter);
     }
   }
-  static void forward(const DevBuf &d, const Route &r, int solver, int a0, int na, int phase_req, int force, int first_only, hipStream_t s) {
+  static void forward(const DevBuf &d, const Route &r, int solver, int a0, int na, int phase_req, int force, int first_only, hipStream_t s, int k1 = 0, int poll_us = 0) {
     if (na <= 0) return;
     const dim3 grid((d.B + 63) / 64, na);
     if (solver == CDDP_HIP_SOLVER_LOGDDP) {
@@ -272,13 +272,13 @@
           if (r.rollout == Route::kGroup2) { hipLaunchKernelGGL((k_forward_ipddp_pcm<Model, Cons, 2>), dim3((d.B + 63) / 64, (na + 1) / 2), dim3(192), 0, s, d, d.P, d.xref_traj, a0, na, phase_req, force); return; }
         }
         if constexpr (PcTwoConsumers<Model, Cons>::value) {
-          if (r.rollout == Route::kTwoConsumers) { hipLaunchKernelGGL((k_forward_ipddp_pc<Model, Cons, false, 2>), grid, dim3(192), 0, s, d, d.P, d.xref_traj, a0, phase_req, force); return; }
-        }
-        hipLaunchKernelGGL((k_forward_ipddp_pc<Model, Cons>), grid, dim3(128), 0, s, d, d.P, d.xref_traj, a0, phase_req, force);
+          if (r.rollout == Route::kTwoConsumers) { hipLaunchKernelGGL((k_forward_ipddp_pc<Model, Cons, false, 2>), grid, dim3(192), 0, s, d, d.P, d.xref_traj, a0, phase_req, force, k1, poll_us); return; }
+        }
+        hipLaunchKernelGGL((k_forward_ipddp_pc<Model, Cons>), grid, dim3(128), 0, s, d, d.P, d.xref_traj, a0, phase_req, force, k1, poll_us);
       } else {
         if constexpr (kTeCoop && Cons::M > 0) {
           if (r.sweep == Route::kCoop) {
-            hipLaunchKernelGGL((k_forward_ipddp_pc<Model, Cons, true>), grid, dim3(128), 0, s, d, d.P, d.xref_traj, a0, phase_req, force);
+            hipLaunchKernelGGL((k_forward_ipddp_pc<Model, Cons, true>), grid, dim3(128), 0, s, d, d.P, d.xref_traj, a0, phase_req, force, 0, 0);
             return;
           }
         }
diff --git a/cddp-cpp_amd/pyapi.py b/cddp-cpp_amd/pyapi.py
--- a/cddp-cpp_amd/pyapi.py
+++ b/cddp-cpp_amd/pyapi.py
@@ -746,7 +746,7 @@
     "cddp_hip_backward_stacks", "cddp_hip_stacks_create_abi", "cddp_hip_stacks_destroy", "cddp_hip_set_stacks", "cddp_hip_set_defect_stack", "cddp_hip_set_control_box", "cddp_hip_set_hessian_stacks", "cddp_hip_set_constraint_stacks",
     "cddp_hip_stacks_backward", "cddp_hip_stacks_last_kernel_ms", "cddp_hip_stacks_last_sweep_form", "cddp_hip_stacks_factor_cache", "cddp_hip_stacks_get_gains", "cddp_hip_stacks_get_constraint_gains",
     "cddp_hip_stacks_get_scalars", "cddp_hip_set_terminal_equality", "cddp_hip_stacks_get_terminal", "cddp_hip_plugin_solve", "cddp_hip_plugin_solve_terminal", "cddp_hip_plugin_set_host_threads", "cddp_hip_plugin_last_stats", "cddp_hip_model_eval", "cddp_hip_set_options", "cddp_hip_set_initial_state", "cddp_hip_forget_solver_state", "cddp_hip_set_duals", "cddp_hip_set_terminal",
-    "cddp_hip_costate_mode", "cddp_hip_costate_redos", "cddp_hip_mpc_advance", "cddp_hip_mpc_run",
+    "cddp_hip_costate_mode", "cddp_hip_costate_redos", "cddp_hip_ls_stage_counts", "cddp_hip_mpc_advance", "cddp_hip_mpc_run",
     "cddp_hip_plant_create", "cddp_hip_plant_destroy", "cddp_hip_plant_step", "cddp_hip_mpc_run_plant", "cddp_hip_track_plan",
     "cddp_hip_field_shape", "cddp_hip_get_field_device", "cddp_hip_get_results_device", "cddp_hip_set_initial_device", "cddp_hip_get_live_slots",
 ]
@@ -792,6 +792,14 @@
 
     def costate_redos(self):
         return int(self.lib.cddp_hip_costate_redos(self.h))
+
+    def ls_stage_counts(self):
+        c = (C.c_longlong * 3)()
+        self.lib.cddp_hip_ls_stage_counts.argtypes = [C.c_void_p, C.POINTER(C.c_longlong)]
+        rc = self.lib.cddp_hip_ls_stage_counts(self.h, c)
+        if rc != 0:
+            raise HipError("cddp_hip_ls_stage_counts failed: %d" % rc)
+        return int(c[0]), int(c[1]), int(c[2])
 
     def set_stream(self, stream_ptr):
         self._check(self.lib.cddp_hip_set_stream(self.h, C.c_void_p(stream_ptr)))
diff --git a/include/cddp_hip.h b/include/cddp_hip.h
--- a/include/cddp_hip.h
+++ b/include/cddp_hip.h
@@ -286,6 +286,7 @@
 int cddp_hip_solve(cddp_hip_handle *h, cddp_hip_stats *stats);
 int cddp_hip_costate_mode(cddp_hip_handle *h);
 int cddp_hip_costate_redos(cddp_hip_handle *h);
+int cddp_hip_ls_stage_counts(cddp_hip_handle *h, long long *counts);
 
 enum cddp_hip_mpc_mode {
   CDDP_HIP_MPC_KEEP_PLAN = 0,
```

Result: faster. 108,200 (median of 6 runs) (+1.7%).
